# fevzibabaoglu/adaptive-edge-aware-jpeg

Hardware: AMD Instinct MI355X
Metric: megapixels/sec encode (Canny+quadtree+DCT+quant), 4K batch (higher is better)
Workload: dtype f32; 1 GPU; 64 x 3840x2160 float32 RGB per GPU, YCbCr, blocks 4-64, quality 40-80 (BASELINE config 4: 512 4K images / 8 GPUs); images_per_gpu=64, height=2160, width=3840, color_space=YCbCr, steps_in_flight=4

## Files before the change

### adaptive_edge_aware_jpeg_amd/_lib.py

```python
import ctypes
import os
import threading

import numpy as np

_HERE = os.path.dirname(os.path.abspath(__file__))
LIB_PATH = os.environ.get("AEJ_LIBRARY") or os.path.join(_HERE, "libaejpeg_hip.so")

SPACE_IDS = {"YCbCr": 0, "YCoCg": 1, "YCoCg-R": 2, "OKLAB": 3, "ICtCp": 4, "ICaCb": 5, "JzAzBz": 6}
CONVERT_IDS = dict(SPACE_IDS, XYZ=7)

AEJ_ERR_ARG, AEJ_ERR_HIP, AEJ_ERR_STATE, AEJ_ERR_CAPACITY, AEJ_ERR_UNSUPPORTED = -1, -2, -3, -4, -5


class AejError(RuntimeError):
    pass


class AejPlan(ctypes.Structure):
    _fields_ = [
        ("batch", ctypes.c_int32), ("H", ctypes.c_int32), ("W", ctypes.c_int32),
        ("layer_h", ctypes.c_int32 * 3), ("layer_w", ctypes.c_int32 * 3), ("root_size", ctypes.c_int32 * 3),
        ("coeff_off", ctypes.c_int64 * 3), ("coeff_stride", ctypes.c_int64),
        ("leaf_off", ctypes.c_int64 * 3), ("leaf_stride", ctypes.c_int64),
        ("state_off", ctypes.c_int64 * 3), ("state_stride", ctypes.c_int64),
        ("workspace_bytes", ctypes.c_uint64),
    ]


_lib = None
_lib_lock = threading.Lock()

HIP_DEFAULT_HW_QUEUES = 4
_hw_queues = HIP_DEFAULT_HW_QUEUES
_hw_queues_source = "HIP default (assumed)"


def _look_at_hw_queues():
    global _hw_queues, _hw_queues_source
    present = os.environ.get("GPU_MAX_HW_QUEUES")
    if present is not None:
        try:
            v = int(present)
        except ValueError:
            v = 0
        if v > 0:
            _hw_queues, _hw_queues_source = v, "GPU_MAX_HW_QUEUES was in the environment when the package was imported"
    return _hw_queues


def configure_hw_queues(want=16):
    global _hw_queues, _hw_queues_source
    import sys
    if os.environ.get("GPU_MAX_HW_QUEUES") is not None:
        return _look_at_hw_queues()
    trusted = "torch" not in sys.modules
    os.environ["GPU_MAX_HW_QUEUES"] = str(int(want))
    if trusted:
        _hw_queues, _hw_queues_source = int(want), "configure_hw_queues() before torch was imported"
        for ctx in _contexts.values():
            ctx.check(ctx.lib.aej_set_hw_queues(ctx.handle, _hw_queues))
    return _hw_queues


def set_hw_queues(n):
    global _hw_queues, _hw_queues_source
    _hw_queues, _hw_queues_source = int(n), "stated by the application (set_hw_queues)"
    for ctx in _contexts.values():
        ctx.check(ctx.lib.aej_set_hw_queues(ctx.handle, _hw_queues))


def hw_queues():
    return _hw_queues, _hw_queues_source


_warned_queue_limited = False


def warn_if_queue_limited(ctx, batch, H, W):
    global _warned_queue_limited
    if _warned_queue_limited:
        return
    sch = ctx.schedule(batch, H, W)
    if sch["limited_by_hw_queues"]:
        _warned_queue_limited = True
        import warnings
        warnings.warn(f"adaptive_edge_aware_jpeg_amd: this call ({batch} x {W}x{H}) would run as more overlapping sub-batches with more hardware "
                      f"queues; the library schedules for {sch['hw_queues']} ({_hw_queues_source}).  Put GPU_MAX_HW_QUEUES=16 into the environment "
                      "(or call adaptive_edge_aware_jpeg_amd.configure_hw_queues()) before `import torch`, or state the runtime's real value with "
                      "set_hw_queues().", RuntimeWarning, stacklevel=3)


_P, _I, _I64, _U64 = ctypes.c_void_p, ctypes.c_int, ctypes.c_int64, ctypes.c_uint64
class CannyParams(ctypes.Structure):
    _fields_ = [("canny_low_ratio", ctypes.c_double), ("canny_high_ratio", ctypes.c_double), ("clahe_clip_limit", ctypes.c_double),
                ("bilateral_sigma_color", ctypes.c_double), ("bilateral_sigma_space", ctypes.c_double), ("use_l2_gradient", ctypes.c_int)]


class JpegDecHuff(ctypes.Structure):
    _fields_ = [("lut", ctypes.c_uint16 * 512), ("maxcode", ctypes.c_int32 * 18), ("valoff", ctypes.c_int32 * 18), ("vals", ctypes.c_uint8 * 256)]


class JfifManyDesc(ctypes.Structure):
    _fields_ = [("src_offset", ctypes.c_int64), ("width", ctypes.c_int32), ("height", ctypes.c_int32), ("quality", ctypes.c_int32),
                ("components", ctypes.c_int32)]


class JpegDecDesc(ctypes.Structure):
    _fields_ = [("width", ctypes.c_int32), ("height", ctypes.c_int32), ("ncomp", ctypes.c_int32), ("hs", ctypes.c_int32), ("vs", ctypes.c_int32),
                ("mcux", ctypes.c_int32), ("mcuy", ctypes.c_int32), ("blocks_per_mcu", ctypes.c_int32), ("restart_interval", ctypes.c_int32),
                ("n_segments", ctypes.c_int32), ("sof", ctypes.c_int32), ("precision16", ctypes.c_int32),
                ("comp_id", ctypes.c_uint8 * 4), ("comp_h", ctypes.c_uint8 * 4), ("comp_v", ctypes.c_uint8 * 4), ("comp_tq", ctypes.c_uint8 * 4),
                ("qt", (ctypes.c_uint16 * 64) * 3), ("dc", JpegDecHuff * 3), ("ac", JpegDecHuff * 3),
                ("scan_offset", ctypes.c_int64), ("scan_length", ctypes.c_int64)]


class JpegProgFrame(ctypes.Structure):
    _fields_ = [("width", ctypes.c_int32), ("height", ctypes.c_int32), ("ncomp", ctypes.c_int32), ("hs", ctypes.c_int32), ("vs", ctypes.c_int32),
                ("mcux", ctypes.c_int32), ("mcuy", ctypes.c_int32), ("blocks_per_mcu", ctypes.c_int32), ("sof", ctypes.c_int32),
                ("precision16", ctypes.c_int32), ("n_scans", ctypes.c_int32), ("n_levels", ctypes.c_int32),
                ("comp_id", ctypes.c_uint8 * 4), ("comp_h", ctypes.c_uint8 * 4), ("comp_v", ctypes.c_uint8 * 4), ("comp_tq", ctypes.c_uint8 * 4),
                ("qt", (ctypes.c_uint16 * 64) * 3)]


class JpegProgScan(ctypes.Structure):
    _fields_ = [("ncomp", ctypes.c_int32), ("comp", ctypes.c_int32 * 4), ("td", ctypes.c_int32 * 4), ("ta", ctypes.c_int32 * 4),
                ("ss", ctypes.c_int32), ("se", ctypes.c_int32), ("ah", ctypes.c_int32), ("al", ctypes.c_int32),
                ("restart_interval", ctypes.c_int32), ("units_x", ctypes.c_int32), ("units_y", ctypes.c_int32),
                ("n_segments", ctypes.c_int32), ("level", ctypes.c_int32), ("dc", JpegDecHuff * 3), ("ac", JpegDecHuff),
                ("data_offset", ctypes.c_int64), ("data_length", ctypes.c_int64)]


class ResampleDesc(ctypes.Structure):
    _fields_ = [("src_offset", ctypes.c_int64), ("dst_offset", ctypes.c_int64), ("src_w", ctypes.c_int32), ("src_h", ctypes.c_int32),
                ("dst_w", ctypes.c_int32), ("dst_h", ctypes.c_int32), ("box", ctypes.c_float * 4), ("filter", ctypes.c_int32),
                ("reduce_x", ctypes.c_int32), ("reduce_y", ctypes.c_int32), ("reduce_box", ctypes.c_int32 * 4), ("reserved", ctypes.c_int32)]


SIGNATURES = {
    "aej_abi_version": (_I, []),
    "aej_create": (_P, [_I, _P]),
    "aej_destroy": (None, [_P]),
    "aej_last_error": (ctypes.c_char_p, [_P]),
    "aej_synchronize": (_I, [_P]),
    "aej_set_stream": (_I, [_P, _P]),
    "aej_get_hysteresis_stats": (_I, [_P, _P]),
    "aej_set_graph_mode": (_I, [_P, _I]),
    "aej_set_sub_batches": (_I, [_P, _I]),
    "aej_set_hw_queues": (_I, [_P, _I]),
    "aej_get_schedule_host": (_I, [_P, _I, _I, _I, _P]),
    "aej_set_option": (_I, [_P, ctypes.c_char_p, _I64]),
    "aej_get_option": (_I, [_P, ctypes.c_char_p, _P]),
    "aej_test_fail_after_stage": (_I, [_P, _I]),
    "aej_encode_batch_begin": (_I, [_P, _P, _I, _I, _I, _I, _P, _P, _P, _P, _P, _P, _U64]),
    "aej_encode_batch_end": (_I, [_P]),
    "aej_get_split_calls": (ctypes.c_int64, [_P]),
    "aej_get_graph_stats": (_I, [_P, _P]),
    "aej_set_profiling": (_I, [_P, _I]),
    "aej_get_stage_ms": (_I, [_P, _P]),
    "aej_stage_name": (ctypes.c_char_p, [_I]),
    "aej_set_settings": (_I, [_P, _I, _I, _I, _P]),
    "aej_encode_plan": (_I, [_P, _I, _I, _I, ctypes.POINTER(AejPlan)]),
    "aej_encode_batch": (_I, [_P, _P, _I, _I, _I, _P, _P, _P, _P, _P, _P, _U64]),
    "aej_encode_batch_u8": (_I, [_P, _P, _I, _I, _I, _P, _P, _P, _P, _P, _P, _U64]),
    "aej_metrics_workspace_bytes": (_U64, [_I, _I, _I]),
    "aej_metrics_batch": (_I, [_P, _P, _P, _I, _I, _I, _I, _P, _P, _U64]),
    "aej_color_convert": (_I, [_P, _I, _P, _P, _I64]),
    "aej_color_planes": (_I, [_P, _P, _I, _I, _I, _P, _P, _P]),
    "aej_canny_workspace_bytes": (_U64, [_I, _I]),
    "aej_canny": (_I, [_P, _P, _I, _I, _P, _P, _P, _P, _U64]),
    "aej_set_canny_params": (_I, [_P, _P]),
    "aej_quadtree_workspace_bytes": (_U64, [_I, _I, _I, _I]),
    "aej_quadtree_capacity": (_I, [_I, _I, _I, _I, ctypes.POINTER(_I64), ctypes.POINTER(_I64), ctypes.POINTER(_I64)]),
    "aej_quadtree": (_I, [_P, _P, _I, _I, _I, _I, _P, _P, _P, _P, _U64]),
    "aej_dct_quant_zigzag": (_I, [_P, _P, _I, _I, _I, _P, _I64, _P, _P]),
    "aej_deflate_stream_bound": (_U64, [_U64]),
    "aej_deflate_workspace_bytes": (_U64, [_P, _I, _I, _I]),
    "aej_deflate_histogram": (_I, [_P, _P, _P, _I, _I, _I, _P, _P, _U64]),
    "aej_deflate_batch": (_I, [_P, _P, _P, _I, _I, _I, _P, _I, _P, _U64, _P, _P, _U64]),
    "aej_deflate_build_tables": (_I, [_P, _P, _P]),
    "aej_pack_u8_levels_host": (_I, [_P, _I64, _P, _I]),
    "aej_decode_workspace_bytes": (_U64, [_P, _I, _I, _I]),
    "aej_decode_batch": (_I, [_P, _P, _P, _P, _I, _I, _I, _P, _P, _U64]),
    "aej_decode_batch_tables": (_I, [_P, _P, _P, _P, _I, _I, _I, _P, _P, _P, _U64]),
    "aej_requantise_batch": (_I, [_P, _P, _P, _P, _I, _I, _I, _I, _P, _P, _U64]),
    "aej_color_convert_inverse": (_I, [_P, _I, _P, _P, _I64]),
    "aej_leaf_positions_host": (_I64, [_P, _I64, _I, _I, _I, _P]),
    "aej_inflate_batch": (_I, [_P, _P, _P, _I, _P, _U64, _P, _P]),
    "aej_decode_headers_workspace_bytes": (_U64, [_P, _I, _I, _I]),
    "aej_decode_headers": (_I, [_P, _P, _P, _P, _I, _I, _I, _P, _P, _P, _P, _U64]),
    "aej_lpips_weights_bytes": (_U64, []),
    "aej_lpips_param_count": (_I64, []),
    "aej_lpips_pack_weights_host": (_I, [_P, _I64, _P]),
    "aej_lpips_features_bytes": (_U64, [_I, _I, _I]),
    "aej_lpips_workspace_bytes": (_U64, [_I, _I, _I]),
    "aej_lpips_features": (_I, [_P, _P, _P, _I, _I, _I, _P, _P, _U64]),
    "aej_lpips_batch": (_I, [_P, _P, _P, _P, _P, _I, _I, _I, _P, _P, _U64]),
    "aej_jfif_workspace_bytes": (_U64, [_I, _I, _I, _I]),
    "aej_jfif_headers_host": (_I, [_I, _I, _I, _P, _I]),
    "aej_jfif_encode_batch": (_I, [_P, _P, _I, _I, _I, _I, _P, _P, _U64, _P, _P, _P, _P, _U64]),
    "aej_jfif_recon_batch": (_I, [_P, _I, _I, _I, _I, _P, _P, _U64]),
    "aej_jfif_workspace_bytes_opt": (_U64, [_I, _I, _I, _I, _I, _I]),
    "aej_jfif_headers_host_opt": (_I, [_I, _I, _I, _I, _P, _I]),
    "aej_jfif_huffman_host": (_I, [_P, _P, _P, _I]),
    "aej_jfif_encode_batch_opt": (_I, [_P, _P, _I, _I, _I, _I, _P, _I, _I, _P, _U64, _P, _P, _P, _P, _U64]),
    "aej_jfif_recon_batch_opt": (_I, [_P, _I, _I, _I, _I, _I, _I, _P, _P, _U64]),
    "aej_jfif_workspace_bytes_prog": (_U64, [_I, _I, _I, _I, _I]),
    "aej_jfif_encode_batch_prog": (_I, [_P, _P, _I, _I, _I, _I, _P, _I, _P, _U64, _P, _P, _P, _P, _U64]),
    "aej_jfif_recon_batch_prog": (_I, [_P, _I, _I, _I, _I, _I, _P, _P, _U64]),
    "aej_test_jfif_prog_scan_host": (_I, [_P, ctypes.c_int64, _I, _I, _I, _I, _P, _U64, _P, _P, _P]),
    "aej_test_jfif_prog_scan": (_I, [_P, _P, ctypes.c_int64, _I, _I, _I, _I, _P, _U64, _P, _P, _P]),
    "aej_jpegdec_parse_host": (_I, [_P, _U64, _P, _P, _I]),
    "aej_jpegdec_workspace_bytes": (_U64, [_P, _P, _I]),
    "aej_jpegdec_batch": (_I, [_P, _P, _I, _P, _U64, _P, _P, _U64, _P, _P, _P, _U64]),
    "aej_jpegdec_sync_rounds": (_I64, [_P]),
    "aej_jpegdec_workspace_bytes_scaled": (_U64, [_P, _P, _I, _P]),
    "aej_jpegdec_batch_scaled": (_I, [_P, _P, _I, _P, _P, _U64, _P, _P, _U64, _P, _P, _P, _U64]),
    "aej_jpegprog_parse_host": (_I, [_P, _U64, _P, _P, _I, _P, _I]),
    "aej_jpegprog_workspace_bytes": (_U64, [_P, _P, _P, _I]),
    "aej_jpegprog_batch": (_I, [_P, _P, _P, _I, _P, _U64, _P, _P, _U64, _P, _P, _P, _U64]),
    "aej_jpegprog_workspace_bytes_scaled": (_U64, [_P, _P, _P, _I, _P]),
    "aej_jpegprog_batch_scaled": (_I, [_P, _P, _P, _I, _P, _P, _U64, _P, _P, _U64, _P, _P, _P, _U64]),
    "aej_jfif_transcode_headers_host": (_I, [_P, _P, _P, _I, _P, _I]),
    "aej_jfif_transcode_workspace_bytes": (_U64, [_P, _P, _I, _P, _P, _I, _I]),
    "aej_jfif_transcode_batch": (_I, [_P, _P, _I, _P, _U64, _P, _P, _P, _I, _P, _U64, _P, _P, _I, _P, _U64, _P, _P, _P, _P, _P, _P, _U64]),
    "aej_jfif_many_workspace_bytes": (_U64, [_P, _P, _I, _I, _I, _I]),
    "aej_jfif_many_encode": (_I, [_P, _P, _I, _P, _U64, _I, _I, _I, _P, _U64, _P, _P, _P, _P, _P, _U64]),
    "aej_jfif_many_coefs_host": (_I64, [_I, _I, _I, _I, _P, _P, _I64]),
    "aej_jfif_headers_grey_host": (_I, [_I, _I, _I, _P, _I]),
    "aej_jfif_many_coefs_grey_host": (_I64, [_I, _I, _I, _P, _P, _I64]),
    "aej_jfif_transform_geometry_host": (_I, [_I, _I, _I, _I, _I, _I, _P]),
    "aej_jfif_transform_coefs_host": (_I64, [_I, _I, _I, _I, _I, _I, _P, _I64, _P, _I64]),
    "aej_jfif_transform_coefs_grey_host": (_I64, [_I, _I, _I, _I, _P, _I64, _P, _I64]),
    "aej_jfif_transform_headers_host": (_I, [_P, _P, _P, _I, _I, _I, _P, _I]),
    "aej_jfif_transform_workspace_bytes": (_U64, [_P, _P, _I, _P, _P, _I, _I, _P, _I]),
    "aej_jfif_transform_batch": (_I, [_P, _P, _I, _P, _U64, _P, _P, _P, _I, _P, _U64, _P, _P, _I, _P, _I, _P, _U64, _P, _P, _P, _P, _P, _P, _U64]),
    "aej_resample_taps_host": (_I, [_I, ctypes.c_float, ctypes.c_float, _I, _I, _P, _P, _I64]),
    "aej_resample_workspace_bytes": (_U64, [_P, _P, _I]),
    "aej_resample_batch": (_I, [_P, _P, _I, _P, _U64, _P, _U64, _P, _U64]),
    "aej_test_jpegprog_coefs": (_I, [_P, _P, _P, _I, _P, _U64, _P, _I, _P, _U64, _P, _P, _U64]),
    "aej_test_jpegprog_coefs_host": (_I, [_P, _P, _P, _U64, _I, _P, _U64]),
    "aej_test_jpegdec_idct_host": (_I, [_P, _P, _I, _P]),
}

INFLATE_STATUS = ["ok", "bad zlib header", "bad block type", "bad code lengths", "invalid literal/length or distance code",
                  "distance too far back", "stored block LEN/NLEN mismatch", "truncated stream", "output over capacity",
                  "Adler-32 mismatch", "bad stream descriptor"]
JPEGDEC_STATUS = ["ok", "truncated scan (it ends before the last MCU)", "bad Huffman code", "coefficient run past 63",
                  "DC category above 11", "restart marker out of sequence, missing or unexpected",
                  "coefficient out of range for an 8-bit JPEG (AC beyond +-1023 or DC outside -1024..1023)"]
HEADER_STATUS = ["ok", "more leaves than the layer holds", "leaf size outside the block-size range of the header",
                 "quadtree header does not tile the layer", "coefficient count does not match the quadtree header", "bad layer descriptor"]


def load_library():
    global _lib
    with _lib_lock:
        if _lib is None:
            if not os.path.exists(LIB_PATH):
                raise AejError(
                    f"{LIB_PATH} is missing: build it with `python -c 'import __graft_entry__ as g; g.build()'` "
                    "(hipcc --offload-arch=gfx950).  There is no CPU fallback.")
            import torch
            lib = ctypes.CDLL(LIB_PATH)
            for name, (res, args) in SIGNATURES.items():
                fn = getattr(lib, name)
                fn.restype = res
                fn.argtypes = args
            _lib = lib
    return _lib


def _torch():
    import torch
    if not torch.cuda.is_available():
        raise AejError("no HIP device visible to PyTorch-ROCm: the adaptive-JPEG encode path runs on the GPU only")
    return torch


class Context:

    def __init__(self, device=0):
        self.torch = _torch()
        self.lib = load_library()
        self.device = self.torch.device("cuda", device if isinstance(device, int) else device.index or 0)
        self.stream = self.torch.cuda.current_stream(self.device).cuda_stream
        self.handle = self.lib.aej_create(self.device.index, ctypes.c_void_p(self.stream))
        if not self.handle:
            raise AejError(self.lib.aej_last_error(None).decode())
        self.check(self.lib.aej_set_hw_queues(self.handle, _hw_queues))
        self.settings_key = None
        self._ws = None

    def check_stream(self):
        cur = self.torch.cuda.current_stream(self.device).cuda_stream
        if cur != self.stream:
            raise AejError(f"context bound to stream {self.stream:#x} used while torch's current stream is {cur:#x}: "
                           "obtain the context with get_context() inside the `torch.cuda.stream(...)` block")

    def __del__(self):
        try:
            if getattr(self, "handle", None):
                self.lib.aej_destroy(self.handle)
                self.handle = None
        except Exception:
# ... 122 lines not shown
```

### adaptive_edge_aware_jpeg_amd/csrc/aej_common.h

```cpp
#pragma once
#include <hip/hip_runtime.h>
#include <stdint.h>

namespace aej {

constexpr int kMaxSizes = 8;
constexpr int kClaheTiles = 4;
constexpr int kHystTile = 64;
constexpr int kBlurTW = 64, kBlurTH = 32;
constexpr int kQtChunk = 256;

struct Geom {
    int B;
    int nl;
    int H, W;
    int h[3], w[3];
    int rh[3], rw[3];
    long long poff[3];
    long long pstride;
    int tiled;
    int ctw[3], cth[3];
    int wpr[3];
    long long bpoff[3];
    long long bpstride;
};

struct QtGeom {
    int bmin, bmax;
    int cell;
    int root[3];
    int ncell[3];
    int ltot[3];
    long long pyr_off[3];
    long long pyr_stride;
    int nchunk[3];
    long long chunk_off[3];
    long long chunk_stride;
    long long coeff_off[3], coeff_stride;
    long long leaf_off[3], leaf_stride;
    long long state_off[3], state_stride;
    long long coeff_cap[3], leaf_cap[3], state_cap[3];
    int nsizes;
    long long work_off[3][kMaxSizes], work_stride[kMaxSizes];
};
struct Tuning {
    int color_strip = 1;
    int color_strip_rows = 0;
    int color_workgroups = 0;
    int planes_row_major = 0;
    int dct64_kernel = 0;
    int dct_small_workgroups = 0;
    int sobel_lds = 0;
    int dct_multi = 1;
    int sobel_xcd = 1;
};

#define AEJ_ZIGZAG_8X8                                                                                                                      \
    0, 1, 8, 16, 9, 2, 3, 10, 17, 24, 32, 25, 18, 11, 4, 5, 12, 19, 26, 33, 40, 48, 41, 34, 27, 20, 13, 6, 7, 14, 21, 28, 35, 42, 49, 56, 57, \
        50, 43, 36, 29, 22, 15, 23, 30, 37, 44, 51, 58, 59, 52, 45, 38, 31, 39, 46, 53, 60, 61, 54, 47, 55, 62, 63

constexpr int kChunkInts = 4 + kMaxSizes;
constexpr int kMaxPlanes = 3072;

constexpr int kMetricBand = 32;

struct LeafWork {
    unsigned xy;
    int coef;
};
__host__ __device__ __forceinline__ LeafWork pack_work(int x, int y, int coef)
{
    LeafWork w;
    w.xy = (unsigned)x | ((unsigned)y << 16);
    w.coef = coef;
    return w;
}
__device__ __forceinline__ int4 unpack_work(int plane, const LeafWork &w) { return make_int4(plane, (int)(w.xy & 0xffffu), (int)(w.xy >> 16), w.coef); }

struct DctTables {
    const float *D[kMaxSizes];
    const int *zzinv[kMaxSizes];
    const int *qm[3][kMaxSizes];
};

__host__ __device__ inline long long plane_elem(int tiled, int w, int y, int x)
{
    return tiled ? ((long long)(y >> 2) * (w >> 2) + (x >> 2)) * 16 + ((y & 3) << 2) + (x & 3) : (long long)y * w + x;
}

__host__ __device__ inline long long bp_index(int y, int xw, int wpr) { return ((long long)(y >> 6) * wpr + xw) * 64 + (y & 63); }
__host__ __device__ inline long long bp_words(int h, int wpr) { return (long long)((h + 63) / 64) * wpr * 64; }

inline int ilog2(int v) { int l = 0; while ((1 << l) < v) l++; return l; }

__device__ __forceinline__ int wave_scan_incl(int v)
{
    v += __builtin_amdgcn_update_dpp(0, v, 0x111, 0xf, 0xf, false);
    v += __builtin_amdgcn_update_dpp(0, v, 0x112, 0xf, 0xf, false);
    v += __builtin_amdgcn_update_dpp(0, v, 0x114, 0xf, 0xf, false);
    v += __builtin_amdgcn_update_dpp(0, v, 0x118, 0xf, 0xf, false);
    v += __builtin_amdgcn_update_dpp(0, v, 0x142, 0xa, 0xf, false);
    v += __builtin_amdgcn_update_dpp(0, v, 0x143, 0xc, 0xf, false);
    return v;
}
__device__ __forceinline__ unsigned wave_max_u32(unsigned v)
{
    auto mx = [](unsigned a, int b) { return a > (unsigned)b ? a : (unsigned)b; };
    v = mx(v, __builtin_amdgcn_update_dpp(0, (int)v, 0x111, 0xf, 0xf, false));
    v = mx(v, __builtin_amdgcn_update_dpp(0, (int)v, 0x112, 0xf, 0xf, false));
    v = mx(v, __builtin_amdgcn_update_dpp(0, (int)v, 0x114, 0xf, 0xf, false));
    v = mx(v, __builtin_amdgcn_update_dpp(0, (int)v, 0x118, 0xf, 0xf, false));
    v = mx(v, __builtin_amdgcn_update_dpp(0, (int)v, 0x142, 0xa, 0xf, false));
    v = mx(v, __builtin_amdgcn_update_dpp(0, (int)v, 0x143, 0xc, 0xf, false));
    return (unsigned)__builtin_amdgcn_readlane((int)v, 63);
}
__device__ __forceinline__ int wave_total(int v) { return __builtin_amdgcn_readlane(wave_scan_incl(v), 63); }

}

#define AEJ_HIP_CHECK(expr)                                                       \
    do {                                                                          \
        hipError_t _e = (expr);                                                   \
        if (_e != hipSuccess) return aej::hip_fail(ctx, _e, #expr, __FILE__, __LINE__); \
    } while (0)
```

### adaptive_edge_aware_jpeg_amd/csrc/aej_ctx.h

```cpp
#pragma once
#include <math.h>
#include <stdarg.h>
#include <stdio.h>
#include <string.h>

#include <algorithm>
#include <atomic>
#include <mutex>
#include <string>
#include <thread>
#include <vector>

#include "../../include/aej.h"
#include "../../include/aej_testing.h"
#include "aej_common.h"
#include "aej_launch.h"

struct aej_pending;
constexpr int kFlagWords = 16;
constexpr int kMaxDevices = 64;
struct aej_ctx {
    int device = 0;
    hipStream_t stream = nullptr;
    std::string err;
    bool has_settings = false;
    int space = 0, bmin = 0, bmax = 0, nsizes = 0;
    void *tables = nullptr;
    const float *d_D[aej::kMaxSizes] = {};
    const int *d_zzinv[aej::kMaxSizes] = {};
    const int *d_zz[aej::kMaxSizes] = {};
    const int *d_qm[3][aej::kMaxSizes] = {};
    int *d_check = nullptr;
    const float *d_space_w = nullptr, *d_color_w = nullptr;
    float *d_bilateral = nullptr;
    aej_canny_params canny = { 0.10, 0.30, 0.75, 75.0, 75.0, 1 };
    int *h_flag = nullptr;
    long long last_hyst_queued = 0;
    bool capturing = false;
    long long n_encode_calls = 0;
    int graph_mode = 0;
    hipStream_t gstream = nullptr;
    hipEvent_t gevent = nullptr;
    struct GraphEntry {
        const void *rgb; void *coeffs, *leaves, *states, *counts, *dct, *ws;
        int batch, H, W, in_u8;
        hipGraphExec_t exec;
        unsigned long long last_use;
    };
    std::vector<GraphEntry> graphs;
    unsigned long long graph_clock = 0, n_graph_launches = 0, n_graph_captures = 0;
    int sub_mode = 0;
    int hw_queues = 4;
    int fail_after = -1;
    static constexpr int kMaxSub = 8;
    int dct_crowded = 0;
    hipStream_t sub_stream[kMaxSub] = {};
    hipEvent_t sub_color_done[kMaxSub] = {}, sub_in = nullptr;
    int *sub_flag[kMaxSub] = {};
    long long n_split_calls = 0;
    int sub_chain = -1;
    int chain_hook = 0;
    hipEvent_t chain_event = nullptr;
    aej::Tuning tune;
    int jd_subseq_bits = 2048;
    long long jd_sync_rounds = 0;
    struct aej_pending *pending = nullptr;
    bool profiling = false;
    hipEvent_t ev[24] = {};
    int ev_stage[24] = {};
    int n_ev = 0;
    float stage_ms[AEJ_N_STAGES] = {};
};

namespace aej {
inline int fail(aej_ctx *ctx, int code, const char *fmt, ...)
{
    char buf[512];
    va_list ap;
    va_start(ap, fmt);
    vsnprintf(buf, sizeof buf, fmt, ap);
    va_end(ap);
    if (ctx) ctx->err = buf;
    return code;
}
int hip_fail(aej_ctx *ctx, hipError_t e, const char *expr, const char *file, int line);

inline bool is_pow2(int v) { return v > 0 && (v & (v - 1)) == 0; }
inline long long align_up(long long v, long long a) { return (v + a - 1) / a * a; }

struct Carver {
    char *base;
    unsigned long long off = 0;
    explicit Carver(void *p) : base(static_cast<char *>(p)) {}
    template <typename T> T *take(long long n)
    {
        off = (off + 255) & ~255ull;
        T *p = base ? reinterpret_cast<T *>(base + off) : nullptr;
        off += (unsigned long long)n * sizeof(T);
        return p;
    }
    unsigned long long bytes() const { return (off + 255) & ~255ull; }
};

}

extern const double kMid[7][3], kScale[7][3];
int check_encode_args(aej_ctx *ctx, int batch, int H, int W);
int make_geom(aej_ctx *ctx, int space, int B, int H, int W, aej::Geom &g);
void make_plane_geom(int H, int W, aej::Geom &g);
int make_qtgeom(aej_ctx *ctx, const aej::Geom &g, int bmin, int bmax, aej::QtGeom &q, bool allow_small_root = false);
int make_geoms(aej_ctx *ctx, int batch, int H, int W, aej::Geom &g, aej::QtGeom &q);
long long big_scratch_floats(int bmax);

bool call_in_flight(const aej_ctx *ctx);
void drop_graphs(aej_ctx *ctx);
void release_encode_state(aej_ctx *ctx);

#define AEJ_TRY(expr) do { const int _rc = (expr); if (_rc) return _rc; } while (0)

inline int refuse_in_flight(aej_ctx *ctx, const char *fn)
{
    return call_in_flight(ctx) ? aej::fail(ctx, AEJ_ERR_STATE, "%s between aej_encode_batch_begin and aej_encode_batch_end", fn) : 0;
}
inline int enter(aej_ctx *ctx, const char *fn) { return ctx ? refuse_in_flight(ctx, fn) : AEJ_ERR_ARG; }
inline int bind_device(aej_ctx *ctx) { AEJ_HIP_CHECK(hipSetDevice(ctx->device)); return 0; }
inline int check_workspace(aej_ctx *ctx, unsigned long long need, uint64_t got)
{
    return need > got ? aej::fail(ctx, AEJ_ERR_CAPACITY, "workspace too small: need %llu bytes, got %llu", need, (unsigned long long)got) : 0;
}
inline int null_buffer(aej_ctx *ctx, const char *fn = nullptr)
{
    return fn ? aej::fail(ctx, AEJ_ERR_ARG, "%s: NULL buffer", fn) : aej::fail(ctx, AEJ_ERR_ARG, "NULL buffer");
}
inline void copy_msg(const std::string &m, char *msg, int msg_capacity)
{
    if (!msg || msg_capacity < 1) return;
    const size_t k = std::min(m.size(), (size_t)msg_capacity - 1);
    memcpy(msg, m.data(), k);
    msg[k] = 0;
}
```

### adaptive_edge_aware_jpeg_amd/csrc/aej_launch.h

```cpp
#pragma once
#include "aej_common.h"

namespace aej {

int launch_color_convert(hipStream_t st, int space, const float *rgb, float *out, long long n);
bool color_planes_can_tile(const Geom &g, int space, bool in_u8, const Tuning &t);
int launch_color_planes(hipStream_t st, int space, const void *rgb, bool in_u8, const Geom &g, const float *mid, const float *scale,
                        float *raw, float *norm, unsigned char *u8, int *tile_hist, const Tuning &t);
struct AreaTabs {
    int mode;
    int isx, isy;
    const int *xoff, *xsi, *yoff, *ysi;
    const float *xal, *yal;
};
int launch_color_planes_generic(hipStream_t st, int space, const void *rgb, bool in_u8, const Geom &g, const float *mid, const float *scale,
                                const AreaTabs &tabs, float *raw, float *norm, unsigned char *u8, int *tile_hist);
void launch_plane_u8(hipStream_t st, const float *plane, const Geom &g, unsigned char *u8, int *tile_hist);

struct CannyBuffers {
    unsigned char *u8a;
    unsigned char *u8b;
    int *tile_hist;
    unsigned char *lut;
    int *blur_hist;
    int *thr;
    unsigned long long *weak;
    unsigned long long *strong;
    int *hflags;
    int *hlist;
    int *pass_count;
    const float *space_w;
    const float *color_w;
    double low_q = 0.10 * 100, high_q = 0.30 * 100;
    double clip_limit = 0.75;
    int l2 = 1;
    unsigned char *dump_clahe, *dump_gauss;
};
constexpr int kHystCounters = 128;
long long hyst_tiles_per_image(const Geom &g);
int hyst_ring_slots(const Geom &g);
void launch_clahe_pad_hist(hipStream_t st, const Geom &g, const CannyBuffers &cb);
void launch_clahe_lut(hipStream_t st, const Geom &g, const CannyBuffers &cb);
void launch_clahe_blur(hipStream_t st, const Geom &g, const CannyBuffers &cb);
void launch_thresholds(hipStream_t st, const Geom &g, const CannyBuffers &cb);
void launch_sobel_nms(hipStream_t st, const Geom &g, const CannyBuffers &cb, const Tuning &t);
void launch_hysteresis(hipStream_t st, const Geom &g, const CannyBuffers &cb);
void launch_zero(hipStream_t st, void *p16, size_t bytes_multiple_of_16);
void launch_bits_to_edge(hipStream_t st, const Geom &g, const unsigned long long *strong, unsigned char *edge01);
void launch_bits_to_map(hipStream_t st, const Geom &g, const unsigned long long *weak, const unsigned long long *strong, unsigned char *map);

struct QtBuffers {
    unsigned char *pyr;
    const unsigned long long *edge_bits;
    int *chunk_cnt;
    unsigned short *lane_code;
    int *leaves;
    unsigned char *states;
    long long *counts;
    LeafWork *work[kMaxSizes];
    int *work_count;
    long long work_cap[kMaxSizes];
    int *overflow;
};
void launch_qt_cells(hipStream_t st, const Geom &g, const QtGeom &q, const unsigned long long *edge_bits, const QtBuffers &qb);
void launch_pack_edge_bits(hipStream_t st, const Geom &g, const unsigned char *edge, unsigned long long *bits);
void launch_qt_count(hipStream_t st, const Geom &g, const QtGeom &q, const QtBuffers &qb);
void launch_qt_scan(hipStream_t st, const Geom &g, const QtGeom &q, const QtBuffers &qb);
void launch_qt_emit(hipStream_t st, const Geom &g, const QtGeom &q, const QtBuffers &qb);

constexpr int kBigBlocks = 128;
constexpr int kMaxBlock = 1024;
constexpr int big_blocks(int S) { return S <= 256 ? kBigBlocks : S == 512 ? 64 : 32; }
constexpr long long big_scratch_floats_for(int S) { return S >= 256 ? (long long)big_blocks(S) * S * S : 0; }
struct DctArgs {
    const float *norm;
    int *coeffs;
    float *dct_f32;
    const LeafWork *work;
    float *scratch;
    const int *work_count;
    int k;
    int nplanes;
    const float *D;
    const int *zzinv;
    const int *qm[3];
    int crowded = 0;
};
int launch_dct(hipStream_t st, int size, const Geom &g, const QtGeom &q, const DctArgs &a, long long max_items, const Tuning &t);
int launch_dct_multi(hipStream_t st, const Geom &g, const QtGeom &q, const DctArgs *args, const long long *max_items);
void launch_work_from_leaves(hipStream_t st, const int *leaves, long long n, int bmin, int plane, LeafWork *const *work, int *work_count);


struct IdctArgs {
    const int *coeffs;
    float *planes;
    const LeafWork *work;
    float *scratch;
    const int *work_count;
    int k, nplanes;
    const float *D;
    const int *zz, *zzinv;
    const int *qm[3];
    float mid[3], scale[3];
};
void launch_work_from_tables(hipStream_t st, const Geom &g, const QtGeom &q, const int *leaves, const long long *counts, LeafWork *const *work,
                             int *work_count, int *bad );
int launch_idct(hipStream_t st, int size, const Geom &g, const QtGeom &q, const IdctArgs &a, long long max_items);
int launch_color_inverse(hipStream_t st, int space, const float *in, float *out, long long n);
int launch_upsample_color(hipStream_t st, int space, const Geom &g, const float *planes, float *rgb);

unsigned long long deflate_stream_bound(unsigned long long raw_bytes);
unsigned long long deflate_workspace_bytes(int batch, const long long *coeff_cap );
void launch_deflate_parse(hipStream_t st, const int *coeffs, const long long *counts, int batch, long long coeff_stride, const long long *coeff_off,
                          const long long *coeff_cap, int *hist, void *workspace);
void launch_deflate(hipStream_t st, const int *coeffs, const long long *counts, int batch, long long coeff_stride, const long long *coeff_off,
                    const long long *coeff_cap, const unsigned *tables , int reuse_parse, unsigned char *out,
                    unsigned long long stream_stride, long long *sizes, void *workspace);

void launch_inflate(hipStream_t st, const unsigned char *src, const long long *desc, int n, unsigned char *dst, long long dst_bytes,
                    long long *out_bytes, int *status);

struct HdrGeom {
    int bmin, bmax;
    int h[3], w[3];
    int proot[3];
    long long leaf_off[3], leaf_span[3], leaf_stride;
    long long coeff_span[3];
};
void launch_headers(hipStream_t st, const unsigned char *states, const long long *desc, const long long *inflated, int nlayers, const HdrGeom &g,
                    unsigned char *codes, int *leaves, long long *counts, int *status);

void launch_requant_check(hipStream_t st, const Geom &g, const QtGeom &q, const int *leaves, const long long *counts, const int *qmats,
                          long long qmat_words, int *bad);
int launch_requant(hipStream_t st, const Geom &g, const QtGeom &q, const float *dct, const int *leaves, const long long *counts, int n_sets,
                   const int *qmats, const int *const *zz, int *out, long long set_stride, int *bad, int blocks_per_plane);

struct MetricParts {
    long long stride;
    int psnr_n;
    long long grey_off, grey_n;
    long long lvl_off[5], lvl_n[5];
};
int metric_prep_blocks(long long npx);
long long ssim_partials(int h, int w);
void launch_metric_prep(hipStream_t st, const float *a, const float *b, int B, long long npx, double *part, long long stride, unsigned char *ga,
                        unsigned char *gb);
void launch_metric_pool_grey(hipStream_t st, const unsigned char *ga, const unsigned char *gb, int B, int H, int W, int f, int hp, int wp, float *xa,
                             float *xb);
void launch_ssim_level(hipStream_t st, bool interleaved, const float *xa, const float *xb, int B, int C, int h, int w, const float *g11, double *part,
                       long long stride, long long off, bool want_ss, float *pool_a = nullptr, float *pool_b = nullptr);
void launch_pool2_rgb(hipStream_t st, const float *ia, const float *ib, int B, int h, int w, int p, int h2, int w2, float *oa, float *ob);
void launch_pool2(hipStream_t st, bool interleaved, const float *in, int B, int C, int h, int w, int p, int h2, int w2, float *out);
void launch_metric_final(hipStream_t st, const double *part, const MetricParts &P, int B, long long npx, long long n_ssim, const long long *n_level, double *out);


constexpr int kLpipsTaps = 5;
constexpr int kLpipsHeadPixels = 256;
struct LpipsLayer { int cin, cinp, cout, k, stride, pad; };
extern const LpipsLayer kLpipsLayers[kLpipsTaps];
struct LpipsGeom {
    int H, W;
    int h[kLpipsTaps], w[kLpipsTaps];
    int ph[2], pw[2];
    long long tap_off[kLpipsTaps];
    long long feat_elems;
    long long x_elems, y_elems;
    int nblk[kLpipsTaps], max_blk;
};
bool lpips_geom(int H, int W, LpipsGeom &g);
long long lpips_param_floats();
long long lpips_packed_floats(long long off[kLpipsTaps][3]);
void lpips_pack_host(const float *params, float *packed);
void launch_lpips(hipStream_t st, const float *wpk, const float *img, int B, const LpipsGeom &g, float *X, float *Y, float *feats_out,
                  const float *feats_a, double *partial, double *out);


constexpr int kJfifBlockWords = 52;
constexpr int kJfifBlockWordsOpt = 53;
constexpr int kJfifHdrMax = 1024;
struct JfifGeom {
    int B, H, W, nq;
    int mcux, mcuy, ybx, yby;
    int yw, yh, cw, ch;
    long long n_mcu, nblk;
    long long stream_words, n_chunks;
    long long plane_bytes;
    int hs, vs, opt, ncomp;
};
struct JfifParams {
    int qt[2][64];
    int hdr_len, dht_off, pad_[2];
    unsigned char hdr[kJfifHdrMax];
};
struct JfifBufs {
    JfifParams *par; int *dct; short *coef; int *lens; long long *boff, *btot; unsigned *stream; int *ffcnt; long long *ffpre, *fftot, *total;
    unsigned char *planes;
    unsigned long long *hist; unsigned *codes; unsigned char *fhdr; int *fhdr_len;
};
bool jfif_geom(int B, int H, int W, int nq, JfifGeom &g, int ss = 2, int opt = 0, int ncomp = 3);
unsigned long long jfif_carve(void *base, const JfifGeom &g, JfifBufs &w);
void jfif_quant_tables(int q, int luma[64], int chroma[64]);
void jfif_params_host(int q, int H, int W, JfifParams &p, int ss = 2, int ncomp = 3);
constexpr int jfif_sof_bytes(int ncomp) { return 10 + 3 * ncomp; }
constexpr int jfif_sos_bytes(int ncomp) { return 8 + 2 * ncomp; }
int jfif_huffman_host(const long long *counts, unsigned char *bits, unsigned char *huffval);
hipError_t launch_jfif_encode(hipStream_t st, const JfifGeom &g, const JfifBufs &w, const JfifParams *par_host, const unsigned char *rgb,
                              unsigned char *out, unsigned long long cap, long long *lengths, long long *offsets);
hipError_t launch_jfif_recon(hipStream_t st, const JfifGeom &g, const JfifBufs &w, unsigned char *rgb_out);
hipError_t launch_jfif_coefs(hipStream_t st, const JfifGeom &g, const JfifBufs &w, const JfifParams *par_host, const unsigned char *rgb);

struct Carver;
unsigned long long jfif_carve_coded(Carver &c, const JfifGeom &g, JfifBufs &w);
hipError_t launch_jfif_entropy(hipStream_t st, const JfifGeom &g, const JfifBufs &w, long long *lengths, long long *offsets);
hipError_t launch_jfif_entropy_annexk(hipStream_t st, const JfifGeom &g, const JfifBufs &w, long long *lengths, long long *offsets);
hipError_t launch_jfif_scatter(hipStream_t st, const JfifGeom &g, const JfifBufs &w, const long long *lengths, const long long *offsets,
                               unsigned char *out, unsigned long long cap);

constexpr int kJfpMaxScans = 10;
constexpr int kJfpPiece = 576;
struct JfpScan {
    int Ss, Se, Ah, Al;
    int comp, tbl;
    long long n, ioff;
    long long woff, wcap, coff;
};
struct JfpGeom {
    int segs, hs, vs, nchroma;
    int mcux, ybx, nscan, ntab;
    int raw, B;
    long long nblk, T, nmax;
    long long stream_words, n_chunks;
    JfpScan sc[kJfpMaxScans];
};
struct JfpBufs {
    unsigned short *flags;
    unsigned long long *pre;
    int *plen, *lens;
    unsigned *stream; int *ffcnt; unsigned long long *ffpre;
// ... 209 lines not shown
```

### adaptive_edge_aware_jpeg_amd/csrc/api.hip

```cpp
#include "aej_ctx.h"

using namespace aej;

int aej::hip_fail(aej_ctx *ctx, hipError_t e, const char *expr, const char *file, int line)
{
    return fail(ctx, AEJ_ERR_HIP, "%s failed: %s (%s:%d)", expr, hipGetErrorString(e), file, line);
}

static const int kRatios[7][3][2] = {
    { { 1, 1 }, { 2, 2 }, { 2, 2 } },
    { { 1, 1 }, { 2, 2 }, { 2, 2 } },
    { { 1, 1 }, { 2, 2 }, { 2, 2 } },
    { { 1, 1 }, { 2, 2 }, { 2, 2 } },
    { { 1, 1 }, { 1, 4 }, { 1, 4 } },
    { { 1, 1 }, { 1, 4 }, { 1, 4 } },
    { { 1, 1 }, { 2, 2 }, { 2, 2 } },
};
const double kMid[7][3] = {
    { 0.5000000037252903, 7.450580596923828e-09, 0.0 }, { 0.5, 0.0, 0.0 }, { 0.5, 0.0, 0.0 },
    { 0.4999999, 0.021152213, -0.056563325 }, { 0.07497266, -0.0008235276, 0.023989676 },
    { 0.07498085, 0.02180194, -0.018250957 }, { 0.0087900255, 0.00048353244, -0.0020741792 },
};
const double kScale[7][3] = {
    { 253.99999810755253, 254.000003784895, 254.0 }, { 254.0, 254.0, 254.0 }, { 254.0, 127.0, 127.0 },
// ... 45 lines not shown
        off += align_up((long long)g.h[l] * g.w[l], 64);
    }
    g.pstride = off;
    fill_clahe_geom(g);
    return 0;
}

void make_plane_geom(int H, int W, Geom &g)
{
    memset(&g, 0, sizeof g);
    g.B = 1; g.nl = 1; g.H = H; g.W = W;
    g.h[0] = H; g.w[0] = W; g.rh[0] = g.rw[0] = 1;
    g.poff[0] = 0;
    g.pstride = align_up((long long)H * W, 64);
    fill_clahe_geom(g);
}

int make_qtgeom(aej_ctx *ctx, const Geom &g, int bmin, int bmax, QtGeom &q, bool allow_small_root)
{
    memset(&q, 0, sizeof q);
    if (!is_pow2(bmin) || !is_pow2(bmax) || bmin > bmax || bmin < 1)
        return fail(ctx, AEJ_ERR_ARG, "block sizes must be powers of two with min <= max (got %d, %d)", bmin, bmax);
    q.bmin = bmin; q.bmax = bmax; q.cell = bmin;
    long long pyr = 0, chunks = 0, co = 0, lo = 0, so = 0;
    for (int l = 0; l < g.nl; l++) {
        int root = root_size_of(g.h[l], g.w[l]);
        if (root < bmin) {
            if (!allow_small_root || g.nl != 1) return fail(ctx, AEJ_ERR_UNSUPPORTED, "layer %d (%dx%d): root %d smaller than min block %d", l, g.h[l], g.w[l], root, bmin);
            q.cell = root;
        }
        q.root[l] = root;
        q.ncell[l] = root / q.cell;
        q.ltot[l] = ilog2(q.ncell[l]);
        if (q.ltot[l] > 14) return fail(ctx, AEJ_ERR_UNSUPPORTED, "quadtree deeper than 14 levels");
        q.pyr_off[l] = pyr;
        long long states = 0;
        for (int j = 0; j <= q.ltot[l]; j++) { long long s = q.ncell[l] >> j; states += s * s; }
        pyr += align_up(states, 256);
        long long nc2 = (long long)q.ncell[l] * q.ncell[l];
        q.nchunk[l] = (int)(nc2 / 256 > 0 ? nc2 / 256 : 1);
        q.chunk_off[l] = chunks;
        chunks += q.nchunk[l];
        int top = bmax < root ? bmax : root;
        long long wc = align_up(g.w[l], top), hc = align_up(g.h[l], top);
        if (wc > root) wc = root;
        if (hc > root) hc = root;
        q.coeff_cap[l] = wc * hc;
        q.leaf_cap[l] = (wc / q.cell) * (hc / q.cell);
        q.state_cap[l] = states;
        q.coeff_off[l] = co; co += align_up(q.coeff_cap[l], 64);
        q.leaf_off[l] = lo;  lo += align_up(q.leaf_cap[l], 16);
        q.state_off[l] = so; so += align_up(q.state_cap[l], 64);
    }
    q.pyr_stride = pyr; q.chunk_stride = chunks;
    q.coeff_stride = co; q.leaf_stride = lo; q.state_stride = so;
    int k = 0;
    for (int s = bmin; s <= bmax && k < kMaxSizes; s *= 2, k++) {
        long long off = 0;
        for (int l = 0; l < g.nl; l++) {
            q.work_off[l][k] = off;
            if (s > q.root[l]) continue;
            int top = bmax < q.root[l] ? bmax : q.root[l];
            long long wc = align_up(g.w[l], top), hc = align_up(g.h[l], top);
            if (wc > q.root[l]) wc = q.root[l];
            if (hc > q.root[l]) hc = q.root[l];
            off += ((wc + s - 1) / s) * ((hc + s - 1) / s);
        }
        q.work_stride[k] = off;
    }
    q.nsizes = k;
    return 0;
}

long long big_scratch_floats(int bmax)
{
    long long m = 0;
    for (int s = 256; s <= bmax; s *= 2) m = std::max(m, big_scratch_floats_for(s));
    return m;
}

int check_encode_args(aej_ctx *ctx, int batch, int H, int W)
{
    if (!ctx) return AEJ_ERR_ARG;
    if (!ctx->has_settings) return fail(ctx, AEJ_ERR_STATE, "aej_set_settings has not been called");
    if (batch < 1 || H < 1 || W < 1) return fail(ctx, AEJ_ERR_ARG, "batch, H, W must be positive");
    if (batch * 3 > kMaxPlanes) return fail(ctx, AEJ_ERR_UNSUPPORTED, "batch %d too large for one call (max %d images)", batch, kMaxPlanes / 3);
    return 0;
}

int make_geoms(aej_ctx *ctx, int batch, int H, int W, Geom &g, QtGeom &q)
{
    AEJ_TRY(make_geom(ctx, ctx->space, batch, H, W, g));
    return make_qtgeom(ctx, g, ctx->bmin, ctx->bmax, q);
}

extern "C" int aej_abi_version(void) { return AEJ_ABI_VERSION; }

extern "C" aej_ctx *aej_create(int device, void *hip_stream)
{
    int n = 0;
    if (hipGetDeviceCount(&n) != hipSuccess || device < 0 || device >= n || device >= kMaxDevices) return nullptr;
    if (hipSetDevice(device) != hipSuccess) return nullptr;
    aej_ctx *ctx = new aej_ctx();
    ctx->device = device;
    ctx->stream = static_cast<hipStream_t>(hip_stream);
    if (hipHostMalloc(reinterpret_cast<void **>(&ctx->h_flag), kFlagWords * sizeof(int), hipHostMallocDefault) != hipSuccess) { delete ctx; return nullptr; }
    return ctx;
}

extern "C" void aej_destroy(aej_ctx *ctx)
{
    if (!ctx) return;
    (void)bind_device(ctx);
    release_encode_state(ctx);
    if (ctx->gstream) (void)hipStreamDestroy(ctx->gstream);
    if (ctx->gevent) (void)hipEventDestroy(ctx->gevent);
    if (ctx->tables) (void)hipFree(ctx->tables);
    if (ctx->d_bilateral) (void)hipFree(ctx->d_bilateral);
    for (int i = 0; i < aej_ctx::kMaxSub; i++) {
        if (ctx->sub_stream[i]) (void)hipStreamDestroy(ctx->sub_stream[i]);
        if (ctx->sub_color_done[i]) (void)hipEventDestroy(ctx->sub_color_done[i]);
        if (ctx->sub_flag[i]) (void)hipHostFree(ctx->sub_flag[i]);
    }
    if (ctx->sub_in) (void)hipEventDestroy(ctx->sub_in);
    if (ctx->h_flag) (void)hipHostFree(ctx->h_flag);
    for (int i = 0; i < 24; i++) if (ctx->ev[i]) (void)hipEventDestroy(ctx->ev[i]);
    delete ctx;
}

extern "C" const char *aej_last_error(aej_ctx *ctx)
{
    if (!ctx) return "aej: no context (aej_create failed: no such HIP device?)";
    return ctx->err.c_str();
}

extern "C" int aej_synchronize(aej_ctx *ctx)
{
    AEJ_TRY(enter(ctx, __func__));
    AEJ_HIP_CHECK(hipStreamSynchronize(ctx->stream));
    return 0;
}

static void zigzag_order(int s, std::vector<int> &zz)
{
    zz.resize((size_t)s * s);
    int i = 0;
    for (int d = 0; d < 2 * s - 1; d++) {
        int lo = d - s + 1 > 0 ? d - s + 1 : 0, hi = d < s - 1 ? d : s - 1;
        if (d % 2) for (int r = lo; r <= hi; r++) zz[i++] = r * s + (d - r);
        else for (int r = hi; r >= lo; r--) zz[i++] = r * s + (d - r);
    }
}

extern "C" int aej_set_settings(aej_ctx *ctx, int space, int bmin, int bmax, const int32_t *qmats_host)
{
    AEJ_TRY(enter(ctx, __func__));
    if (space < 0 || space > 6) return fail(ctx, AEJ_ERR_ARG, "Unsupported color space id: %d", space);
    if (!is_pow2(bmin) || !is_pow2(bmax) || bmin > bmax || bmin < 2)
        return fail(ctx, AEJ_ERR_ARG, "block size range (%d, %d): powers of two with 2 <= min <= max required", bmin, bmax);
    if (bmax > kMaxBlock)
        return fail(ctx, AEJ_ERR_UNSUPPORTED, "block size range (%d, %d): no kernel for blocks above %d", bmin, bmax, kMaxBlock);
    if (ilog2(bmax) - ilog2(bmin) + 1 > kMaxSizes)
        return fail(ctx, AEJ_ERR_UNSUPPORTED, "block size range (%d, %d) spans more than %d sizes", bmin, bmax, kMaxSizes);
    if (!qmats_host) return fail(ctx, AEJ_ERR_ARG, "qmats_host is NULL");
    AEJ_TRY(bind_device(ctx));
    int nsizes = 0;
    for (int s = bmin; s <= bmax; s *= 2) nsizes++;
    std::vector<char> blob;
    auto put = [&](const void *p, size_t bytes) {
        size_t o = (blob.size() + 255) & ~(size_t)255;
        blob.resize(o + bytes);
        memcpy(blob.data() + o, p, bytes);
        return o;
    };
    size_t oD[kMaxSizes], oZ[kMaxSizes], oZf[kMaxSizes], oQ[3][kMaxSizes];
    int k = 0;
    size_t qpos = 0;
    std::vector<size_t> qoff_layer_size;
    for (int s = bmin; s <= bmax; s *= 2, k++) {
        std::vector<float> D((size_t)s * s);
        for (int u = 0; u < s; u++) {
            double alpha = u == 0 ? sqrt(1.0 / (double)s) : sqrt(2.0 / (double)s);
            for (int n = 0; n < s; n++) D[(size_t)u * s + n] = (float)(alpha * cos(3.14159265358979323846 * (double)(2 * n + 1) * (double)u / (2.0 * (double)s)));
        }
        oD[k] = put(D.data(), D.size() * 4);
        std::vector<int> zz, inv((size_t)s * s);
        zigzag_order(s, zz);
        for (int i = 0; i < s * s; i++) inv[zz[i]] = i;
        oZ[k] = put(inv.data(), inv.size() * 4);
        oZf[k] = put(zz.data(), zz.size() * 4);
    }
    for (int l = 0; l < 3; l++) {
        k = 0;
        for (int s = bmin; s <= bmax; s *= 2, k++) {
            for (int i = 0; i < s * s; i++)
                if (qmats_host[qpos + i] < 1) return fail(ctx, AEJ_ERR_ARG, "quantisation matrix entries must be >= 1");
            oQ[l][k] = put(qmats_host + qpos, (size_t)s * s * 4);
            qpos += (size_t)s * s;
        }
    }
    const int zero_words[64] = {};
    const size_t oCheck = put(zero_words, sizeof zero_words);
    drop_graphs(ctx);
    if (ctx->tables) { AEJ_HIP_CHECK(hipStreamSynchronize(ctx->stream)); AEJ_HIP_CHECK(hipFree(ctx->tables)); ctx->tables = nullptr; }
    AEJ_HIP_CHECK(hipMalloc(&ctx->tables, blob.size()));
    AEJ_HIP_CHECK(hipMemcpy(ctx->tables, blob.data(), blob.size(), hipMemcpyHostToDevice));
    char *base = static_cast<char *>(ctx->tables);
    for (int i = 0; i < kMaxSizes; i++) {
        ctx->d_D[i] = nullptr; ctx->d_zzinv[i] = nullptr; ctx->d_zz[i] = nullptr;
        for (int l = 0; l < 3; l++) ctx->d_qm[l][i] = nullptr;
    }
    for (int i = 0; i < nsizes; i++) {
        ctx->d_D[i] = reinterpret_cast<const float *>(base + oD[i]);
        ctx->d_zzinv[i] = reinterpret_cast<const int *>(base + oZ[i]);
        ctx->d_zz[i] = reinterpret_cast<const int *>(base + oZf[i]);
        for (int l = 0; l < 3; l++) ctx->d_qm[l][i] = reinterpret_cast<const int *>(base + oQ[l][i]);
    }
    ctx->d_check = reinterpret_cast<int *>(base + oCheck);
    ctx->space = space; ctx->bmin = bmin; ctx->bmax = bmax; ctx->nsizes = nsizes;
    ctx->has_settings = true;
    return 0;
}

extern "C" int aej_set_canny_params(aej_ctx *ctx, const aej_canny_params *p)
{
    AEJ_TRY(enter(ctx, __func__));
    const aej_canny_params def = { 0.10, 0.30, 0.75, 75.0, 75.0, 1 };
    const aej_canny_params v = p ? *p : def;
    if (!(v.canny_low_ratio >= 0.0 && v.canny_low_ratio <= 1.0 && v.canny_high_ratio >= 0.0 && v.canny_high_ratio <= 1.0))
        return fail(ctx, AEJ_ERR_ARG, "Canny threshold ratios must lie in [0, 1] (np.percentile takes 0..100)");
    if (!(v.clahe_clip_limit == v.clahe_clip_limit) || !(v.bilateral_sigma_color == v.bilateral_sigma_color) || !(v.bilateral_sigma_space == v.bilateral_sigma_space))
        return fail(ctx, AEJ_ERR_ARG, "NaN Canny hyper-parameter");
    const bool tables_change = v.bilateral_sigma_color != ctx->canny.bilateral_sigma_color || v.bilateral_sigma_space != ctx->canny.bilateral_sigma_space;
    ctx->canny = v;
    drop_graphs(ctx);
    if (tables_change) { ctx->d_color_w = nullptr; ctx->d_space_w = nullptr; }
    return 0;
}

extern "C" int aej_get_hysteresis_stats(aej_ctx *ctx, int64_t *out_host)
{
    if (!ctx || !out_host) return AEJ_ERR_ARG;
    out_host[0] = ctx->n_encode_calls;
    out_host[1] = ctx->last_hyst_queued;
    return 0;
}

extern "C" int aej_set_graph_mode(aej_ctx *ctx, int mode)
{
    if (!ctx || mode < 0 || mode > 2) return AEJ_ERR_ARG;
    AEJ_TRY(refuse_in_flight(ctx, __func__));
    ctx->graph_mode = mode;
    if (mode == 0) drop_graphs(ctx);
    return 0;
}

extern "C" int aej_set_sub_batches(aej_ctx *ctx, int n)
{
    if (!ctx || n < 0 || n > aej_ctx::kMaxSub) return AEJ_ERR_ARG;
    ctx->sub_mode = n;
    return 0;
}

extern "C" int64_t aej_get_split_calls(aej_ctx *ctx) { return ctx ? (int64_t)ctx->n_split_calls : -1; }

extern "C" int aej_set_hw_queues(aej_ctx *ctx, int n)
{
    if (!ctx || n < 1) return AEJ_ERR_ARG;
    ctx->hw_queues = n;
    return 0;
}

namespace {
struct OptionDef { const char *name; int aej::Tuning::*field; int aej_ctx::*ctx_field; long long lo, hi; bool drops_graphs; };
const OptionDef kOptions[] = {
    { "color_strip", &aej::Tuning::color_strip, nullptr, 0, 1, true },
    { "color_strip_rows", &aej::Tuning::color_strip_rows, nullptr, 0, 64, true },
    { "color_workgroups", &aej::Tuning::color_workgroups, nullptr, 0, 1 << 16, true },
    { "planes_row_major", &aej::Tuning::planes_row_major, nullptr, 0, 1, true },
    { "dct64_kernel", &aej::Tuning::dct64_kernel, nullptr, 0, 4, true },
    { "dct_small_workgroups", &aej::Tuning::dct_small_workgroups, nullptr, 0, 1 << 16, true },
    { "sobel_lds", &aej::Tuning::sobel_lds, nullptr, 0, 1, true },
    { "sobel_xcd", &aej::Tuning::sobel_xcd, nullptr, 0, 1, true },
    { "dct_multi", &aej::Tuning::dct_multi, nullptr, 0, 1, true },
    { "sub_chain", nullptr, &aej_ctx::sub_chain, -1, 3, false },
    { "jpegdec_subseq_bits", nullptr, &aej_ctx::jd_subseq_bits, 32, 1 << 20, false },
};
const OptionDef *find_option(const char *name)
{
    if (!name) return nullptr;
    for (const OptionDef &o : kOptions) if (!strcmp(o.name, name)) return &o;
    return nullptr;
}
}

extern "C" int aej_set_option(aej_ctx *ctx, const char *name, int64_t value)
{
    AEJ_TRY(enter(ctx, __func__));
    const OptionDef *o = find_option(name);
    if (!o) return fail(ctx, AEJ_ERR_ARG, "aej_set_option: unknown option '%s'", name ? name : "(null)");
    if (value < o->lo || value > o->hi || (o->field == &aej::Tuning::dct64_kernel && value != 0 && value != 1 && value != 4))
        return fail(ctx, AEJ_ERR_ARG, "aej_set_option: %s = %lld outside its range [%lld, %lld]", name, (long long)value, o->lo, o->hi);
    if (o->field) ctx->tune.*(o->field) = (int)value;
    else ctx->*(o->ctx_field) = (int)value;
    if (o->drops_graphs) drop_graphs(ctx);
    return 0;
}

extern "C" int aej_get_option(aej_ctx *ctx, const char *name, int64_t *value_host)
{
    if (!ctx || !value_host) return AEJ_ERR_ARG;
    const OptionDef *o = find_option(name);
    if (!o) return fail(ctx, AEJ_ERR_ARG, "aej_get_option: unknown option '%s'", name ? name : "(null)");
    *value_host = o->field ? ctx->tune.*(o->field) : ctx->*(o->ctx_field);
    return 0;
}

extern "C" int aej_test_fail_after_stage(aej_ctx *ctx, int stage)
{
    if (!ctx || stage < -1 || stage >= AEJ_N_STAGES) return AEJ_ERR_ARG;
    ctx->fail_after = stage;
    return 0;
}

extern "C" int aej_get_graph_stats(aej_ctx *ctx, int64_t *out_host)
{
    if (!ctx || !out_host) return AEJ_ERR_ARG;
    out_host[0] = (int64_t)ctx->n_graph_launches;
    out_host[1] = (int64_t)ctx->n_graph_captures;
    out_host[2] = (int64_t)ctx->graphs.size();
    return 0;
}

extern "C" int aej_set_stream(aej_ctx *ctx, void *hip_stream)
{
    AEJ_TRY(enter(ctx, __func__));
    hipStream_t s = static_cast<hipStream_t>(hip_stream);
    if (s == ctx->stream) return 0;
    AEJ_TRY(bind_device(ctx));
    AEJ_HIP_CHECK(hipStreamSynchronize(ctx->stream));
    ctx->stream = s;
    return 0;
}

extern "C" int aej_set_profiling(aej_ctx *ctx, int enable)
{
    AEJ_TRY(enter(ctx, __func__));
    ctx->profiling = enable != 0;
    return 0;
}

extern "C" int aej_get_stage_ms(aej_ctx *ctx, float *ms_host)
{
    if (!ctx || !ms_host) return AEJ_ERR_ARG;
    for (int i = 0; i < AEJ_N_STAGES; i++) ms_host[i] = ctx->stage_ms[i];
    return 0;
}

extern "C" const char *aej_stage_name(int i)
{
    static const char *names[AEJ_N_STAGES] = { "clear", "color_planes", "clahe_lut", "clahe_blur", "thresholds", "sobel_nms",
                                               "hysteresis", "quadtree", "dct2", "dct4", "dct8", "dct16", "dct32", "dct64", "dct128", "dct256", "dct512", "dct1024" };
    return i >= 0 && i < AEJ_N_STAGES ? names[i] : "";
}
```

### adaptive_edge_aware_jpeg_amd/csrc/api_encode.hip

```cpp
#include "aej_ctx.h"

using namespace aej;

static void mark(aej_ctx *ctx, int stage)
{
    if (!ctx->profiling || ctx->n_ev >= 24) return;
    if (!ctx->ev[ctx->n_ev] && hipEventCreate(&ctx->ev[ctx->n_ev]) != hipSuccess) return;
    ctx->ev_stage[ctx->n_ev] = stage;
    (void)hipEventRecord(ctx->ev[ctx->n_ev], ctx->stream);
    ctx->n_ev++;
}

static int injected_failure(aej_ctx *ctx, int stage)
{
    if (ctx->fail_after != stage) return 0;
    ctx->fail_after = -1;
    ctx->err = std::string("injected failure after stage ") + aej_stage_name(stage);
    return AEJ_ERR_STATE;
}

static void collect_marks(aej_ctx *ctx)
{
    for (int i = 0; i < AEJ_N_STAGES; i++) ctx->stage_ms[i] = 0.f;
    for (int i = 1; i < ctx->n_ev; i++) {
// ... 134 lines not shown
{
    hipStream_t st = ctx->stream;
    if (ctx->capturing) launch_zero(st, w.zero_begin, (size_t)(w.zero_end - w.zero_begin));
    else AEJ_HIP_CHECK(hipMemsetAsync(w.zero_begin, 0, (size_t)(w.zero_end - w.zero_begin), st));
    w.qb.edge_bits = edge_bits;
    launch_qt_cells(st, g, q, edge_bits, w.qb);
    launch_qt_count(st, g, q, w.qb);
    launch_qt_scan(st, g, q, w.qb);
    launch_qt_emit(st, g, q, w.qb);
    AEJ_HIP_CHECK(hipGetLastError());
    return 0;
}

static void area_tab(int ssize, int dsize, double scale, std::vector<int> &off, std::vector<int> &si, std::vector<float> &alpha)
{
    off.assign((size_t)dsize + 1, 0); si.clear(); alpha.clear();
    for (int dx = 0; dx < dsize; dx++) {
        double fsx1 = dx * scale, fsx2 = fsx1 + scale;
        double cell = scale < ssize - fsx1 ? scale : ssize - fsx1;
        int sx1 = (int)ceil(fsx1), sx2 = (int)floor(fsx2);
        if (sx2 > ssize - 1) sx2 = ssize - 1;
        if (sx1 > sx2) sx1 = sx2;
        off[dx] = (int)si.size();
        if (sx1 - fsx1 > 1e-3) { si.push_back(sx1 - 1); alpha.push_back((float)((sx1 - fsx1) / cell)); }
        for (int sx = sx1; sx < sx2; sx++) { si.push_back(sx); alpha.push_back((float)(1.0 / cell)); }
        if (fsx2 - sx2 > 1e-3) {
            double a = fsx2 - sx2;
            if (a > 1.) a = 1.;
            if (a > cell) a = cell;
            si.push_back(sx2); alpha.push_back((float)(a / cell));
        }
    }
    off[dsize] = (int)si.size();
}

static long long area_tab_ints(const Geom &g)
{
    return 2LL * (g.w[1] + 1 + g.h[1] + 1) + 2LL * (g.W + 2 * g.w[1] + 2) + 2LL * (g.H + 2 * g.h[1] + 2) + 64;
}

static bool planes_fast_ok(const Geom &g)
{
    bool ok = (g.W % 4) == 0 && (g.H % 2) == 0;
    for (int l = 1; l < 3; l++) ok = ok && g.h[l] * g.rh[l] == g.H && g.w[l] * g.rw[l] == g.W;
    return ok;
}

static int run_color_planes(aej_ctx *ctx, const void *rgb, bool in_u8, const Geom &g, float *raw, float *norm, unsigned char *u8, int *hist,
                            int *tab_ws)
{
    float mid[3], scale[3];
    for (int i = 0; i < 3; i++) { mid[i] = (float)kMid[ctx->space][i]; scale[i] = (float)kScale[ctx->space][i]; }
    if (planes_fast_ok(g)) {
        Tuning t = ctx->tune;
        if (t.color_workgroups == 0 && ctx->dct_crowded && ctx->space < 3) t.color_workgroups = 224;
        if (launch_color_planes(ctx->stream, ctx->space, rgb, in_u8, g, mid, scale, raw, norm, u8, hist, t)) return fail(ctx, AEJ_ERR_ARG, "bad colour space");
        return 0;
    }
    AreaTabs t;
    memset(&t, 0, sizeof t);
    double sx = 1.0 / ((double)g.w[1] / (double)g.W), sy = 1.0 / ((double)g.h[1] / (double)g.H);
    int isx = (int)lrint(sx), isy = (int)lrint(sy);
    bool fast = fabs(sx - isx) < 2.220446049250313e-16 && fabs(sy - isy) < 2.220446049250313e-16;
    t.isx = isx; t.isy = isy;
    if (fast) t.mode = (isx == 2 && isy == 2) ? 0 : 1;
    else {
        t.mode = 2;
        if (!tab_ws) return fail(ctx, AEJ_ERR_STATE, "no workspace for the INTER_AREA tables");
        std::vector<int> xoff, xsi, yoff, ysi;
        std::vector<float> xal, yal;
        area_tab(g.W, g.w[1], sx, xoff, xsi, xal);
        area_tab(g.H, g.h[1], sy, yoff, ysi, yal);
        std::vector<int> blob;
        auto put_i = [&](const std::vector<int> &v) { size_t o = blob.size(); blob.insert(blob.end(), v.begin(), v.end()); return o; };
        auto put_f = [&](const std::vector<float> &v) { size_t o = blob.size(); blob.resize(o + v.size()); memcpy(blob.data() + o, v.data(), v.size() * 4); return o; };
        size_t o1 = put_i(xoff), o2 = put_i(xsi), o3 = put_f(xal), o4 = put_i(yoff), o5 = put_i(ysi), o6 = put_f(yal);
        if ((long long)blob.size() > area_tab_ints(g)) return fail(ctx, AEJ_ERR_CAPACITY, "INTER_AREA tables larger than reserved");
        AEJ_HIP_CHECK(hipMemcpyAsync(tab_ws, blob.data(), blob.size() * 4, hipMemcpyHostToDevice, ctx->stream));
        AEJ_HIP_CHECK(hipStreamSynchronize(ctx->stream));
        t.xoff = tab_ws + o1; t.xsi = tab_ws + o2; t.xal = reinterpret_cast<const float *>(tab_ws + o3);
        t.yoff = tab_ws + o4; t.ysi = tab_ws + o5; t.yal = reinterpret_cast<const float *>(tab_ws + o6);
    }
    if (launch_color_planes_generic(ctx->stream, ctx->space, rgb, in_u8, g, mid, scale, t, raw, norm, u8, hist)) return fail(ctx, AEJ_ERR_ARG, "bad colour space");
    return 0;
}

struct EncodeWs {
    float *big;
    float *norm;
    int *area_tabs;
    CannyWs canny;
    QtWs qt;
    unsigned long long bytes;
};

static void carve_encode(void *base, const Geom &g, const QtGeom &q, EncodeWs &w)
{
    Carver c(base);
    w.norm = c.take<float>((long long)g.B * g.pstride);
    w.area_tabs = c.take<int>(area_tab_ints(g));
    carve_canny(c, g, w.canny);
    carve_qt(c, g, q, true, w.qt);
    w.big = big_scratch_floats(q.bmax) ? c.take<float>(big_scratch_floats(q.bmax)) : nullptr;
    w.bytes = c.bytes();
}

static unsigned long long sub_ws_bytes(Geom g, const QtGeom &q, int nsub)
{
    g.B = (g.B + nsub - 1) / nsub;
    EncodeWs w;
    carve_encode(nullptr, g, q, w);
    return w.bytes;
}

extern "C" int aej_encode_plan(aej_ctx *ctx, int batch, int H, int W, aej_plan *plan)
{
    AEJ_TRY(check_encode_args(ctx, batch, H, W));
    if (!plan) return fail(ctx, AEJ_ERR_ARG, "plan is NULL");
    Geom g;
    QtGeom q;
    AEJ_TRY(make_geoms(ctx, batch, H, W, g, q));
    EncodeWs w;
    carve_encode(nullptr, g, q, w);
    memset(plan, 0, sizeof *plan);
    plan->batch = batch; plan->H = H; plan->W = W;
    for (int l = 0; l < 3; l++) {
        plan->layer_h[l] = g.h[l]; plan->layer_w[l] = g.w[l]; plan->root_size[l] = q.root[l];
        plan->coeff_off[l] = q.coeff_off[l]; plan->leaf_off[l] = q.leaf_off[l]; plan->state_off[l] = q.state_off[l];
    }
    plan->coeff_stride = q.coeff_stride; plan->leaf_stride = q.leaf_stride; plan->state_stride = q.state_stride;
    plan->workspace_bytes = w.bytes;
    for (int n = 2; n <= aej_ctx::kMaxSub && n <= batch; n++)
        plan->workspace_bytes = std::max<uint64_t>(plan->workspace_bytes, sub_ws_bytes(g, q, n) * (unsigned long long)n);
    return 0;
}

constexpr long long kGraphAutoPixels = 8LL << 20;

static int enqueue_back(aej_ctx *ctx, const Geom &g, const QtGeom &q, EncodeWs &w, int32_t *coeffs, float *dct_f32)
{
    hipStream_t st = ctx->stream;
    AEJ_TRY(run_quadtree(ctx, g, q, w.qt, w.canny.cb.strong));
    mark(ctx, AEJ_STAGE_QUADTREE);
    DctArgs args[kMaxSizes];
    int k = 0;
    for (int s = q.bmin; s <= q.bmax; s *= 2, k++) {
        DctArgs &a = args[k];
        a.norm = w.norm; a.coeffs = coeffs; a.dct_f32 = dct_f32;
        a.work = w.qt.qb.work[k]; a.work_count = w.qt.qb.work_count; a.k = k; a.nplanes = g.B * 3;
        a.scratch = w.big;
        a.D = ctx->d_D[k]; a.zzinv = ctx->d_zzinv[k];
        a.crowded = ctx->dct_crowded;
        for (int l = 0; l < 3; l++) a.qm[l] = ctx->d_qm[l][k];
    }
    const bool one_launch = ctx->tune.dct_multi && !ctx->profiling && (long long)g.B * g.H * g.W <= kGraphAutoPixels;
    if (!(one_launch && launch_dct_multi(st, g, q, args, w.qt.qb.work_cap) == 0)) {
        k = 0;
        for (int s = q.bmin; s <= q.bmax; s *= 2, k++) {
            if (launch_dct(st, s, g, q, args[k], w.qt.qb.work_cap[k], ctx->tune)) return fail(ctx, AEJ_ERR_UNSUPPORTED, "no DCT kernel for block size %d with %d planes", s, args[k].nplanes);
            mark(ctx, AEJ_STAGE_DCT_2 + ilog2(s) - 1);
        }
    }
    AEJ_HIP_CHECK(hipGetLastError());
    return 0;
}

static int enqueue_readback(aej_ctx *ctx, EncodeWs &w)
{
    AEJ_HIP_CHECK(hipMemcpyAsync(ctx->h_flag, w.qt.qb.overflow, sizeof(int), hipMemcpyDeviceToHost, ctx->stream));
    AEJ_HIP_CHECK(hipMemcpyAsync(ctx->h_flag + 1, w.canny.cb.pass_count + 32 , sizeof(int), hipMemcpyDeviceToHost, ctx->stream));
    return 0;
}

constexpr size_t kMaxGraphs = 8;

static int encode_graph(aej_ctx *ctx, const void *rgb, bool in_u8, const Geom &g, const QtGeom &q, EncodeWs &w, int32_t *coeffs, int32_t *leaves,
                        uint8_t *states, int64_t *counts, float *dct_f32, void *workspace, bool &used)
{
    used = false;
    if (!ctx->gstream) {
        AEJ_HIP_CHECK(hipStreamCreateWithFlags(&ctx->gstream, hipStreamNonBlocking));
        AEJ_HIP_CHECK(hipEventCreateWithFlags(&ctx->gevent, hipEventDisableTiming));
    }
    aej_ctx::GraphEntry *hit = nullptr;
    for (auto &e : ctx->graphs)
        if (e.rgb == rgb && e.coeffs == coeffs && e.leaves == leaves && e.states == states && e.counts == counts && e.dct == dct_f32 && e.ws == workspace &&
            e.batch == g.B && e.H == g.H && e.W == g.W && e.in_u8 == (int)in_u8) { hit = &e; break; }
    hipStream_t user = ctx->stream;
    if (!hit) {
        if (ctx->graphs.size() >= kMaxGraphs) {
            size_t lru = 0;
            for (size_t i = 1; i < ctx->graphs.size(); i++) if (ctx->graphs[i].last_use < ctx->graphs[lru].last_use) lru = i;
            if (ctx->graphs[lru].exec) (void)hipGraphExecDestroy(ctx->graphs[lru].exec);
            ctx->graphs.erase(ctx->graphs.begin() + (long)lru);
        }
        ctx->graphs.push_back({ rgb, coeffs, leaves, states, counts, dct_f32, workspace, g.B, g.H, g.W, (int)in_u8, nullptr, ++ctx->graph_clock });
        return 0;
    }
    if (!hit->exec) {
        hipGraph_t graph = nullptr;
        ctx->stream = ctx->gstream;
        ctx->capturing = true;
        hipError_t e = hipStreamBeginCapture(ctx->gstream, hipStreamCaptureModeThreadLocal);
        int rc = e == hipSuccess ? 0 : hip_fail(ctx, e, "hipStreamBeginCapture", __FILE__, __LINE__);
        if (!rc) rc = clear_canny_ws(ctx, w.canny);
        if (!rc) rc = run_color_planes(ctx, rgb, in_u8, g, nullptr, w.norm, w.canny.cb.u8a, w.canny.cb.tile_hist, w.area_tabs);
        if (!rc) {
            hipStream_t st = ctx->stream;
            launch_clahe_pad_hist(st, g, w.canny.cb);
            launch_clahe_lut(st, g, w.canny.cb);
            launch_clahe_blur(st, g, w.canny.cb);
            launch_thresholds(st, g, w.canny.cb);
            launch_sobel_nms(st, g, w.canny.cb, ctx->tune);
            launch_hysteresis(st, g, w.canny.cb);
            rc = enqueue_back(ctx, g, q, w, coeffs, dct_f32);
        }
        hipError_t e2 = e == hipSuccess ? hipStreamEndCapture(ctx->gstream, &graph) : hipSuccess;
        ctx->stream = user;
        ctx->capturing = false;
        if (rc || e2 != hipSuccess || !graph) {
            if (graph) (void)hipGraphDestroy(graph);
            (void)hipGetLastError();
            return rc ? rc : 0;
        }
        hipGraphExec_t exec = nullptr;
        e = hipGraphInstantiate(&exec, graph, nullptr, nullptr, 0);
        (void)hipGraphDestroy(graph);
        if (e != hipSuccess || !exec) { (void)hipGetLastError(); return 0; }
        hit->exec = exec;
        ctx->n_graph_captures++;
    }
    hit->last_use = ++ctx->graph_clock;
    AEJ_HIP_CHECK(hipEventRecord(ctx->gevent, user));
    AEJ_HIP_CHECK(hipStreamWaitEvent(ctx->gstream, ctx->gevent, 0));
    AEJ_HIP_CHECK(hipGraphLaunch(hit->exec, ctx->gstream));
    ctx->stream = ctx->gstream;
    const int rb = enqueue_readback(ctx, w);
    ctx->stream = user;
    if (rb) return rb;
    AEJ_HIP_CHECK(hipStreamSynchronize(ctx->gstream));
    ctx->n_graph_launches++;
    used = true;
    return 0;
}

static int sub_batches(const aej_ctx *ctx, const Geom &g, int hw_queues, bool as_if_unprofiled = false)
{
    if (ctx->sub_mode == 1 || (ctx->profiling && !as_if_unprofiled) || ctx->graph_mode == 2 || !planes_fast_ok(g)) return 1;
    int n = ctx->sub_mode;
    if (n == 0) {
        const long long px = (long long)g.B * g.H * g.W;
        if (hw_queues >= 8) {
            n = (px >= (384LL << 20) && g.B >= 16) ? 4 : (px >= (64LL << 20) && g.B >= 8) ? 2 : 1;
        } else {
            bool alone;
            { std::lock_guard<std::mutex> lock(g_chain_mutex); alone = g_calls_in_flight[ctx->device] == 0; }
            n = (alone && px >= (64LL << 20) && g.B >= 8) ? 2 : 1;
        }
    }
    if (n > aej_ctx::kMaxSub) n = aej_ctx::kMaxSub;
    if (n > g.B) n = g.B;
    return n;
}

struct EncodePart { Geom g; EncodeWs w; bool whole_call = false; int32_t *coeffs = nullptr; float *dct = nullptr; hipStream_t stream = nullptr; int *flag = nullptr; bool used = false; };
struct aej_pending {
    bool active = false, complete = false;
    QtGeom q;
    std::vector<EncodePart> parts;
};

bool call_in_flight(const aej_ctx *ctx) { return ctx->pending && ctx->pending->active; }

void release_encode_state(aej_ctx *ctx)
{
    if (call_in_flight(ctx)) {
        (void)hipDeviceSynchronize();
        std::lock_guard<std::mutex> lock(g_chain_mutex);
        if (g_calls_in_flight[ctx->device] > 0) g_calls_in_flight[ctx->device]--;
    }
    delete ctx->pending;
    ctx->pending = nullptr;
    {
        std::lock_guard<std::mutex> lock(g_chain_mutex);
        for (int i = 0; i < aej_ctx::kMaxSub; i++)
            if (ctx->sub_color_done[i] && g_last_color_done[ctx->device] == ctx->sub_color_done[i]) g_last_color_done[ctx->device] = nullptr;
    }
    drop_graphs(ctx);
}

static aej_pending &pending_of(aej_ctx *ctx)
{
    if (!ctx->pending) ctx->pending = new aej_pending;
    return *ctx->pending;
}

static int enqueue_part(aej_ctx *ctx, EncodePart &p, const QtGeom &q, const void *rgb, bool in_u8, hipEvent_t done)
{
    int rc;
    mark(ctx, -1);
    AEJ_TRY(clear_canny_ws(ctx, p.w.canny));
    mark(ctx, AEJ_STAGE_CLEAR);
    const bool chain = ctx->sub_chain && done && !ctx->profiling;
    const int chain_mode = ctx->sub_chain > 0 ? ctx->sub_chain : 1;
    if (chain) {
        std::lock_guard<std::mutex> lock(g_chain_mutex);
// ... 203 lines not shown
    AEJ_TRY(bind_device(ctx));
    Geom g;
    AEJ_TRY(make_geom(ctx, ctx->space, batch, H, W, g));
    int *tabs = nullptr;
    if (!planes_fast_ok(g)) AEJ_HIP_CHECK(hipMalloc(reinterpret_cast<void **>(&tabs), (size_t)area_tab_ints(g) * 4));
    const int rc = run_color_planes(ctx, rgb, false, g, planes_raw, planes_norm, planes_u8, nullptr, tabs);
    if (tabs) { (void)hipStreamSynchronize(ctx->stream); (void)hipFree(tabs); }
    if (rc) return rc;
    AEJ_HIP_CHECK(hipGetLastError());
    return 0;
}

extern "C" uint64_t aej_canny_workspace_bytes(int H, int W)
{
    if (H < 1 || W < 1) return 0;
    Geom g;
    make_plane_geom(H, W, g);
    Carver c(nullptr);
    CannyWs w;
    carve_canny(c, g, w);
    return c.bytes();
}

extern "C" int aej_canny(aej_ctx *ctx, const float *plane, int H, int W, uint8_t *edge, uint8_t *stages, int32_t *thresholds,
                         void *workspace, uint64_t workspace_bytes)
{
    AEJ_TRY(enter(ctx, __func__));
    if (H < 1 || W < 1) return fail(ctx, AEJ_ERR_ARG, "Input array must be a 2D.");
    if (!plane || !edge || !workspace) return null_buffer(ctx);
    if (workspace_bytes < aej_canny_workspace_bytes(H, W)) return fail(ctx, AEJ_ERR_CAPACITY, "workspace too small");
    AEJ_TRY(bind_device(ctx));
    AEJ_TRY(ensure_canny_tables(ctx));
    Geom g;
    make_plane_geom(H, W, g);
    Carver c(workspace);
    CannyWs w;
    carve_canny(c, g, w);
    apply_canny_params(ctx, w.cb);
    long long n = (long long)H * W;
    if (stages) { w.cb.dump_clahe = stages + n; w.cb.dump_gauss = stages + 2 * n; }
    AEJ_TRY(clear_canny_ws(ctx, w));
    launch_plane_u8(ctx->stream, plane, g, w.cb.u8a, w.cb.tile_hist);
    hipStream_t st = ctx->stream;
    if (stages) AEJ_HIP_CHECK(hipMemcpyAsync(stages, w.cb.u8a, n, hipMemcpyDeviceToDevice, st));
    launch_clahe_pad_hist(st, g, w.cb);
    launch_clahe_lut(st, g, w.cb);
    launch_clahe_blur(st, g, w.cb);
    if (stages) AEJ_HIP_CHECK(hipMemcpyAsync(stages + 3 * n, w.cb.u8b, n, hipMemcpyDeviceToDevice, st));
    launch_thresholds(st, g, w.cb);
    if (thresholds) AEJ_HIP_CHECK(hipMemcpyAsync(thresholds, w.cb.thr, 2 * sizeof(int), hipMemcpyDeviceToDevice, st));
    launch_sobel_nms(st, g, w.cb, ctx->tune);
    Geom ge = g;
    ge.pstride = n;
    if (stages) launch_bits_to_map(st, ge, w.cb.weak, w.cb.strong, stages + 4 * n);
    launch_hysteresis(st, g, w.cb);
    launch_bits_to_edge(st, ge, w.cb.strong, edge);
    AEJ_HIP_CHECK(hipGetLastError());
    AEJ_HIP_CHECK(hipStreamSynchronize(st));
    return 0;
}

extern "C" int aej_quadtree_capacity(int H, int W, int min_size, int max_size, int64_t *leaf_cap, int64_t *state_cap, int64_t *coeff_cap)
{
    if (H < 1 || W < 1) return AEJ_ERR_ARG;
    Geom g;
    make_plane_geom(H, W, g);
    QtGeom q;
    AEJ_TRY(make_qtgeom(nullptr, g, min_size, max_size, q, true));
    if (leaf_cap) *leaf_cap = q.leaf_cap[0];
    if (state_cap) *state_cap = q.state_cap[0];
    if (coeff_cap) *coeff_cap = q.coeff_cap[0];
    return 0;
}

extern "C" uint64_t aej_quadtree_workspace_bytes(int H, int W, int min_size, int max_size)
{
    if (H < 1 || W < 1) return 0;
    Geom g;
    make_plane_geom(H, W, g);
    QtGeom q;
    if (make_qtgeom(nullptr, g, min_size, max_size, q, true)) return 0;
    Carver c(nullptr);
    QtWs w;
    carve_qt(c, g, q, false, w);
    c.take<unsigned long long>(g.bpstride);
    return c.bytes();
}

extern "C" int aej_quadtree(aej_ctx *ctx, const uint8_t *edge, int H, int W, int min_size, int max_size, int32_t *leaves,
                            uint8_t *states, int64_t *counts, void *workspace, uint64_t workspace_bytes)
{
    AEJ_TRY(enter(ctx, __func__));
    if (H < 1 || W < 1) return fail(ctx, AEJ_ERR_ARG, "Input array must be a 2D with a single channel.");
    if (!edge || !leaves || !states || !counts || !workspace) return null_buffer(ctx);
    AEJ_TRY(bind_device(ctx));
    Geom g;
    make_plane_geom(H, W, g);
    g.pstride = (long long)H * W;
    QtGeom q;
    AEJ_TRY(make_qtgeom(ctx, g, min_size, max_size, q, true));
    Carver c(workspace);
    QtWs w;
    carve_qt(c, g, q, false, w);
    unsigned long long *bits = c.take<unsigned long long>(g.bpstride);
    if (c.bytes() > workspace_bytes) return fail(ctx, AEJ_ERR_CAPACITY, "workspace too small");
    w.qb.leaves = leaves; w.qb.states = states; w.qb.counts = reinterpret_cast<long long *>(counts);
    launch_pack_edge_bits(ctx->stream, g, edge, bits);
    AEJ_TRY(run_quadtree(ctx, g, q, w, bits));
    AEJ_HIP_CHECK(hipMemcpyAsync(ctx->h_flag, w.qb.overflow, sizeof(int), hipMemcpyDeviceToHost, ctx->stream));
    AEJ_HIP_CHECK(hipStreamSynchronize(ctx->stream));
    if (*ctx->h_flag) return fail(ctx, AEJ_ERR_CAPACITY, "leaf/state capacity exceeded");
    return 0;
}

extern "C" int aej_dct_quant_zigzag(aej_ctx *ctx, const float *norm, int H, int W, int layer, const int32_t *leaves, int64_t n_leaves,
                                    int32_t *coeffs, float *dct_f32)
{
    AEJ_TRY(enter(ctx, __func__));
    if (!ctx->has_settings) return fail(ctx, AEJ_ERR_STATE, "aej_set_settings has not been called");
    if (H < 1 || W < 1 || layer < 0 || layer > 2 || n_leaves < 0) return fail(ctx, AEJ_ERR_ARG, "bad argument");
    if (H > 65535 || W > 65535) return fail(ctx, AEJ_ERR_UNSUPPORTED, "plane %dx%d: sides above 65535 pixels are not built", H, W);
    if (n_leaves == 0) return 0;
    if (!norm || !leaves || !coeffs) return null_buffer(ctx);
    AEJ_TRY(bind_device(ctx));
    hipStream_t st = ctx->stream;
    Geom g;
    memset(&g, 0, sizeof g);
    g.B = 1; g.nl = 3; g.H = H; g.W = W;
    for (int l = 0; l < 3; l++) { g.h[l] = H; g.w[l] = W; g.rh[l] = g.rw[l] = 1; g.poff[l] = 0; }
    g.pstride = (long long)H * W;
    QtGeom q;
    memset(&q, 0, sizeof q);
    q.bmin = ctx->bmin; q.bmax = ctx->bmax; q.cell = ctx->bmin; q.nsizes = ctx->nsizes;
    char *scratch = nullptr;
    size_t list_bytes = (size_t)n_leaves * sizeof(LeafWork);
    size_t total = 256 + (size_t)ctx->nsizes * ((list_bytes + 255) & ~(size_t)255);
    const size_t big_off = total;
    total += (size_t)big_scratch_floats(ctx->bmax) * sizeof(float);
    AEJ_HIP_CHECK(hipMalloc(reinterpret_cast<void **>(&scratch), total));
    int *work_count = reinterpret_cast<int *>(scratch);
    LeafWork *work[kMaxSizes] = {};
    for (int k = 0; k < ctx->nsizes; k++) work[k] = reinterpret_cast<LeafWork *>(scratch + 256 + (size_t)k * ((list_bytes + 255) & ~(size_t)255));
    hipError_t e = hipMemsetAsync(scratch, 0, 256, st);
    if (e == hipSuccess) {
        launch_work_from_leaves(st, leaves, n_leaves, ctx->bmin, layer, work, work_count);
        int k = 0;
        for (int s = ctx->bmin; s <= ctx->bmax; s *= 2, k++) {
            DctArgs a;
            a.norm = norm; a.coeffs = coeffs; a.dct_f32 = dct_f32;
            a.work = work[k]; a.work_count = work_count; a.k = k; a.nplanes = 3;
            a.scratch = big_scratch_floats(ctx->bmax) ? reinterpret_cast<float *>(scratch + big_off) : nullptr;
            a.D = ctx->d_D[k]; a.zzinv = ctx->d_zzinv[k];
            for (int l = 0; l < 3; l++) a.qm[l] = ctx->d_qm[l][k];
            if (launch_dct(st, s, g, q, a, n_leaves, ctx->tune)) { e = hipErrorInvalidValue; break; }
        }
        if (e == hipSuccess) e = hipGetLastError();
        if (e == hipSuccess) e = hipStreamSynchronize(st);
    }
    (void)hipFree(scratch);
    if (e != hipSuccess) return fail(ctx, AEJ_ERR_HIP, "aej_dct_quant_zigzag: %s", hipGetErrorString(e));
    return 0;
}

extern "C" int aej_get_schedule_host(aej_ctx *ctx, int batch, int H, int W, int32_t *out_host)
{
    AEJ_TRY(check_encode_args(ctx, batch, H, W));
    if (!out_host) return fail(ctx, AEJ_ERR_ARG, "out_host is NULL");
    Geom g;
    AEJ_TRY(make_geom(ctx, ctx->space, batch, H, W, g));
    const int n = sub_batches(ctx, g, ctx->hw_queues), n_wide = sub_batches(ctx, g, 16);
    out_host[0] = ctx->hw_queues;
    out_host[1] = n;
    out_host[2] = (ctx->hw_queues < 8 && n_wide > n) ? 1 : 0;
    out_host[3] = 0;
    return 0;
}
```

### adaptive_edge_aware_jpeg_amd/csrc/dct.hip

```cpp
#include "aej_common.h"
#include "aej_launch.h"
#include "aej_bigblock.h"
#include "aej_mfma.h"
#include "aej_quant.h"
#include <stdlib.h>

namespace aej {


__device__ __forceinline__ int reflect_pad_idx(int i, int n)
{
    if (i < n) return i;
    if (n <= 1) return 0;
    int p = 2 * (n - 1);
    int j = i % p;
    return j >= n ? p - j : j;
}

template <int S>
__device__ __forceinline__ int zigzag_pos(int r, int c)
{
    const int d = r + c;
    if (d < S) {
        const int before = d * (d + 1) / 2;
// ... 505 lines not shown
                for (int s = 0; s < 4; s++) x[s] = (row0 + (long long)s * (w >> 2) * 16)[lane_tiled];
            } else {
                const float *row0 = src + ((long long)dz * w + dy);
                const unsigned lane_rm = (unsigned)(gq * w + i);
#pragma unroll
                for (int s = 0; s < 4; s++) x[s] = (row0 + (long long)s * 4 * w)[lane_rm];
            }
        } else {
            const int hc = min(S, h - dz), wc = min(S, w - dy);
            const int col = dy + reflect_pad_idx(i, wc);
#pragma unroll
            for (int s = 0; s < 4; s++) x[s] = src[plane_elem(TILED ? 1 : 0, w, dz + reflect_pad_idx(4 * s + gq, hc), col)];
        }
    };
    Desc d0 = landed(fetch(item)), d1, d2;
    float x0[4], x1[4], x2[4];
    load_x(d0, x0);
    d1 = landed(fetch(item + 4));
    Desc dv = fetch(item + 8);
    load_x(d1, x1);
    auto step = [&](const float (&x_cur)[4], const Desc &d_cur, float (&x_fill)[4], Desc &d_fill) {
        d_fill = landed(dv);
        dv = fetch(item + 12);
        load_x(d_fill, x_fill);
        const int b = d_cur.plane / 3, layer = d_cur.plane - b * 3;
        floatx4 pacc = { 0.f, 0.f, 0.f, 0.f };
#pragma unroll
        for (int s = 0; s < 4; s++) pacc = __builtin_amdgcn_mfma_f32_16x16x4f32(x_cur[s], dB[s], pacc, 0, 0, 0);
        const auto p02 = __builtin_amdgcn_permlane32_swap(__float_as_uint(pacc[0]), __float_as_uint(pacc[2]), false, false);
        const auto p13 = __builtin_amdgcn_permlane32_swap(__float_as_uint(pacc[1]), __float_as_uint(pacc[3]), false, false);
        const unsigned p02a = p02[0], p02b = p02[1], p13a = p13[0], p13b = p13[1];
        const auto q01 = __builtin_amdgcn_permlane16_swap(p02a, p13a, false, false);
        const auto q23 = __builtin_amdgcn_permlane16_swap(p02b, p13b, false, false);
        const unsigned t0 = q01[0], t1 = q01[1], t2 = q23[0], t3 = q23[1];
        const float t[4] = { __uint_as_float(t0), __uint_as_float(t1), __uint_as_float(t2), __uint_as_float(t3) };
        floatx4 y = { 0.f, 0.f, 0.f, 0.f };
#pragma unroll
        for (int s = 0; s < 4; s++) y = __builtin_amdgcn_mfma_f32_16x16x4f32(t[s], dB[s], y, 0, 0, 0);
        const long long out_base = (long long)b * q.coeff_stride + sel(layer, lcoff[0], lcoff[1], lcoff[2]) + d_cur.coef;
        if (WANT_DCT) {
#pragma unroll
            for (int r = 0; r < 4; r++) a.dct_f32[out_base + (4 * gq + r) * S + i] = y[r];
        }
        const floatx4 qf = *reinterpret_cast<const floatx4 *>(&sQf[layer * SS + lane * 4]), rq = *reinterpret_cast<const floatx4 *>(&sQr[layer * SS + lane * 4]);
        const float ymax = __builtin_fmaxf(__builtin_fmaxf(__builtin_fabsf(y[0]), __builtin_fabsf(y[1])), __builtin_fmaxf(__builtin_fabsf(y[2]), __builtin_fabsf(y[3])));
        if (!slow_q && !__any(!(ymax < 131072.0f))) {
            float kf[4], rem[4];
            unsigned long long fix = 0;
#pragma unroll
            for (int r = 0; r < 4; r++) {
                kf[r] = __builtin_rintf(y[r] * rq[r]);
                rem[r] = __builtin_fmaf(-kf[r], qf[r], y[r]);
                const float ar = __builtin_fabsf(rem[r]);
                fix |= __builtin_amdgcn_ballot_w64(ar + ar >= qf[r]);
            }
            int ki[4];
#pragma unroll
            for (int r = 0; r < 4; r++) ki[r] = (int)kf[r];
            if (fix != 0) {
#pragma unroll
                for (int r = 0; r < 4; r++) {
                    const float ar = __builtin_fabsf(rem[r]), h = 0.5f * qf[r];
                    if (ar > h || (ar == h && (ki[r] & 1))) ki[r] += rem[r] > 0.f ? 1 : -1;
                }
            }
#pragma unroll
            for (int r = 0; r < 4; r++) out_slab[zz[r]] = ki[r];
        } else {
#pragma unroll
            for (int r = 0; r < 4; r++) out_slab[zz[r]] = quantise_f64(y[r], qm_exact(a, layer, (4 * gq + r) * S + i));
        }
        const int4 o = reinterpret_cast<const int4 *>(out_slab)[lane];
        reinterpret_cast<int4 *>(a.coeffs + out_base)[lane] = o;
    };
    while (true) {
        step(x0, d0, x2, d2); item += 4; if (item >= last) break;
        step(x1, d1, x0, d0); item += 4; if (item >= last) break;
        step(x2, d2, x1, d1); item += 4; if (item >= last) break;
    }
}
template <bool WANT_DCT>
__device__ __forceinline__ void dct16_body(const Geom &g, const QtGeom &q, const DctArgs &a, long long max_items, unsigned bid, unsigned nb)
{
    __shared__ Dct16Lds L;
    if (g.tiled) dct16_impl<WANT_DCT, true>(L, g, q, a, max_items, bid, nb);
    else dct16_impl<WANT_DCT, false>(L, g, q, a, max_items, bid, nb);
}
template <bool WANT_DCT>
__global__ __launch_bounds__(256) void k_dct16_mfma(Geom g, QtGeom q, DctArgs a, long long max_items)
{
    dct16_body<WANT_DCT>(g, q, a, max_items, blockIdx.x, gridDim.x);
}

template <int S, bool WANT_DCT>
__global__ __launch_bounds__(256) void k_dct_big(Geom g, QtGeom q, DctArgs a, long long max_items)
{
    __shared__ BigTileLds L;
    __shared__ LayerTab lt;
    extern __shared__ int s_pref[];
    dct_prologue(g, q, a, s_pref, lt);
    long long count = s_pref[a.nplanes];
    if (count > max_items) count = max_items;
    const long long wstride = q.work_stride[a.k];
    float *T = a.scratch + (long long)blockIdx.x * S * S;
    for (long long item = blockIdx.x; item < count; item += gridDim.x) {
        const int4 cur = fetch_item(a, wstride, lt, s_pref, item);
        const int b = cur.x / 3, layer = cur.x - b * 3;
        const int w = lt.w[layer], h = lt.h[layer];
        const float *src = a.norm + (long long)b * g.pstride + lt.poff[layer];
        const int hc = min(S, h - cur.z), wc = min(S, w - cur.y);
        const float *D = a.D;
        big_product<S>(L,
            [&](int i, int k) { return D[i * S + k]; },
            [&](int k, int j) { return src[plane_elem(g.tiled, w, cur.z + reflect_pad_idx(k, hc), cur.y + reflect_pad_idx(j, wc))]; },
            [&](int i, int j, float v) { T[i * S + j] = v; });
        big_scratch_sync();
        const long long out_base = (long long)b * q.coeff_stride + lt.coff[layer] + cur.w;
        const int *qm = a.qm[layer];
        big_product<S>(L,
            [&](int i, int k) { return T[i * S + k]; },
            [&](int k, int j) { return D[j * S + k]; },
            [&](int i, int j, float v) {
                const int ridx = i * S + j;
                if (WANT_DCT) a.dct_f32[out_base + ridx] = v;
                a.coeffs[out_base + a.zzinv[ridx]] = quantise(v, qm ? qm[ridx] : 1);
            });
        big_scratch_sync();
    }
}

__device__ __forceinline__ void glds16(const float *g, float *lds_wave_base)
{
    unsigned keep;
    const unsigned dst = __builtin_amdgcn_readfirstlane((unsigned)(size_t)lds_wave_base);
    asm volatile("s_mov_b32 %0, m0\n\ts_mov_b32 m0, %2\n\ts_nop 0\n\tglobal_load_lds_dwordx4 %1, off\n\ts_mov_b32 m0, %0"
                 : "=&s"(keep) : "v"(g), "s"(dst) : "memory");
}
__device__ __forceinline__ void glds4(const float *g, float *lds_wave_base)
{
    unsigned keep;
    const unsigned dst = __builtin_amdgcn_readfirstlane((unsigned)(size_t)lds_wave_base);
    asm volatile("s_mov_b32 %0, m0\n\ts_mov_b32 m0, %2\n\ts_nop 0\n\tglobal_load_lds_dword %1, off\n\ts_mov_b32 m0, %0"
                 : "=&s"(keep) : "v"(g), "s"(dst) : "memory");
}

template <int S>
struct MfmaCfg {
    static constexpr int NT = S / 32;
    static constexpr int TPW = S == 128 ? 2 : 1;
    static constexpr int NWAVES = NT * NT / TPW;
    static constexpr int NTHREADS = NWAVES * 64;
    static constexpr int MINW = S == 32 ? 4 : S == 64 ? 3 : 2;
    static constexpr int NXB = S == 128 ? 1 : 2;
};

__device__ __forceinline__ void glds16_s(const float *base_uniform, unsigned lane_byte_off, float *lds_wave_base)
{
    unsigned keep;
    const unsigned dst = __builtin_amdgcn_readfirstlane((unsigned)(size_t)lds_wave_base);
    const unsigned long long b = (unsigned long long)(size_t)base_uniform;
    const unsigned blo = __builtin_amdgcn_readfirstlane((unsigned)b), bhi = __builtin_amdgcn_readfirstlane((unsigned)(b >> 32));
    const unsigned long long sb = ((unsigned long long)bhi << 32) | blo;
    asm volatile("s_mov_b32 %0, m0\n\ts_mov_b32 m0, %2\n\ts_nop 0\n\tglobal_load_lds_dwordx4 %1, %3\n\ts_mov_b32 m0, %0"
                 : "=&s"(keep) : "v"(lane_byte_off), "s"(dst), "s"(sb) : "memory");
}

template <int S, int NWAVES>
struct XOffsets { unsigned off[S * S / 256 / NWAVES]; int w; };

template <int S, int NWAVES>
__device__ __forceinline__ void dct_x_offsets(XOffsets<S, NWAVES> &xo, int w, int tiled, int wave, int lane)
{
    constexpr int ROWS = 256 / S;
#pragma unroll
    for (int t = 0; t < S * S / 256 / NWAVES; t++) {
        const int chunk = t * NWAVES + wave;
        const int r = chunk * ROWS + lane / (S / 4), c = (lane % (S / 4)) * 4;
        xo.off[t] = (unsigned)plane_elem(tiled, w, r, c) * 4u;
    }
    xo.w = w;
}

template <int S, int NWAVES>
__device__ __forceinline__ void dct_load_x(const float *src, int w, int h, int tiled, const int4 &d, float *sX, int wave, int lane, XOffsets<S, NWAVES> &xo)
{
    constexpr int SS = S * S;
    const int hc = min(S, h - d.z), wc = min(S, w - d.y);
    if (hc == S && wc == S && (w & 3) == 0) {
        if (xo.w != w) dct_x_offsets<S, NWAVES>(xo, w, tiled, wave, lane);
        const float *leaf = src + plane_elem(tiled, w, d.z, d.y);
#pragma unroll
        for (int t = 0; t < SS / 256 / NWAVES; t++) glds16_s(leaf, xo.off[t], sX + (t * NWAVES + wave) * 256);
    } else {
#pragma unroll 4
        for (int t = 0; t < SS / 64 / NWAVES; t++) {
            const int chunk = t * NWAVES + wave;
            const int idx = chunk * 64 + lane;
            const int r = idx / S, c = idx - r * S;
            glds4(src + plane_elem(tiled, w, d.z + reflect_pad_idx(r, hc), d.y + reflect_pad_idx(c, wc)), sX + chunk * 64);
        }
    }
}

__device__ __forceinline__ void lds_barrier() { asm volatile("s_waitcnt lgkmcnt(0)\n\ts_barrier" ::: "memory"); }
template <int N> __device__ __forceinline__ void wait_vmem_but() { asm volatile("s_waitcnt vmcnt(%0)" :: "n"(N) : "memory"); }


template <int S, bool WANT_DCT>
__device__ __forceinline__ void dct_mfma_leaves(const Geom &g, const QtGeom &q, const DctArgs &a, long long max_items, const LeafWork *__restrict__ work ,
                                                unsigned bid, unsigned nb)
{
    using C = MfmaCfg<S>;
    constexpr int NT = C::NT, TPW = C::TPW, NWAVES = C::NWAVES, NTHREADS = C::NTHREADS;
    constexpr int SS = S * S;
    constexpr int NXB = C::NXB;
    constexpr int NCOPY = SS / (NTHREADS * 4);
    constexpr int NYOUNG = NCOPY + (WANT_DCT ? 16 * TPW : 0);
    static_assert(NYOUNG < 60, "vmcnt is a 6-bit counter");
    extern __shared__ __attribute__((aligned(16))) float smem[];
    float *sXb = smem;
    float *sP = smem + NXB * SS;
    int4 *s_desc = reinterpret_cast<int4 *>(smem + (NXB + 1) * SS);
    LayerTab &lt = *reinterpret_cast<LayerTab *>(s_desc + 2 * kDescChunk);
    int *s_pref = reinterpret_cast<int *>(s_desc + 2 * kDescChunk) + (sizeof(LayerTab) + 3) / 4;
    const int tid = threadIdx.x;
    const int wave = tid >> 6, lane = tid & 63;
    const int wj = wave % NT, wi0 = wave / NT;
    const int J0 = wj * 32;
    const int li = lane & 31, lh = lane >> 5;

    float dreg[S / 2];
#pragma unroll
    for (int s = 0; s < S / 2; s++) dreg[s] = a.D[(J0 + li) * S + 2 * s + lh];

    dct_prologue(g, q, a, s_pref, lt);
#pragma unroll
    for (int s = 0; s < S / 2; s++) asm volatile("" : "+v"(dreg[s]));
    long long count = s_pref[a.nplanes];
    if (count > max_items) count = max_items;
    const long long wstride = q.work_stride[a.k];
    const long long step = nb;
    long long item = bid;
    auto load_chunk = [&](long long c) {
        if (tid < kDescChunk) {
            const long long it = (long long)bid + (c * kDescChunk + tid) * step;
            int4 d = make_int4(0, 0, 0, 0);
            if (it < count) d = fetch_item(a, wstride, lt, s_pref, it);
            s_desc[(c & 1) * kDescChunk + tid] = d;
        }
    };
    load_chunk(0);
    load_chunk(1);
    __syncthreads();
    long long k = 0;
    struct LeafU { int plane, x, y, coef; };
    auto uniform = [](const int4 &d) {
        return LeafU{ __builtin_amdgcn_readfirstlane(d.x), __builtin_amdgcn_readfirstlane(d.y), __builtin_amdgcn_readfirstlane(d.z),
                      __builtin_amdgcn_readfirstlane(d.w) };
    };
    auto plane_of = [&](const LeafU &d, int &b, int &layer, int &w, int &h, const float *&src) {
        b = d.plane / 3;
        layer = d.plane - 3 * b;
        w = layer == 0 ? g.w[0] : layer == 1 ? g.w[1] : g.w[2];
        h = layer == 0 ? g.h[0] : layer == 1 ? g.h[1] : g.h[2];
        const long long poff = layer == 0 ? g.poff[0] : layer == 1 ? g.poff[1] : g.poff[2];
        src = a.norm + (long long)b * g.pstride + poff;
    };
    LeafU cur = uniform(s_desc[0]), nxt = uniform(s_desc[1]);
    int pb = 0;
    XOffsets<S, NWAVES> xo;
    xo.w = -1;
    if (NXB == 2 && item < count) {
        int b0, l0, w0, h0;
        const float *src0;
        plane_of(cur, b0, l0, w0, h0, src0);
        dct_load_x<S, NWAVES>(src0, w0, h0, g.tiled, make_int4(cur.plane, cur.x, cur.y, cur.coef), sXb, wave, lane, xo);
        wait_vmem_but<0>();
    }
    float qf[TPW][16];
    int q_layer = -1;
    bool q_slow = false;
    for (; item < count; item += step) {
        int b, layer, lw, lhh;
        const float *src;
        plane_of(cur, b, layer, lw, lhh, src);
        const long long coff = layer == 0 ? q.coeff_off[0] : layer == 1 ? q.coeff_off[1] : q.coeff_off[2];
        const long long out_base = (long long)b * q.coeff_stride + coff + cur.coef;
        float *sX = sXb + pb * SS;
        if (S == 128 || layer != q_layer) {
            const int *qm = layer == 0 ? a.qm[0] : layer == 1 ? a.qm[1] : a.qm[2];
            int qmax = 0;
#pragma unroll
            for (int t = 0; t < TPW; t++)
#pragma unroll
                for (int r = 0; r < 16; r++) {
                    const int qi = qm[((wi0 + t * (NT / TPW)) * 32 + (r & 3) + 8 * (r >> 2) + 4 * lh) * S + J0 + li];
                    qmax = max(qmax, qi);
                    qf[t][r] = (float)qi;
                }
            q_slow = __any(qmax > (1 << 22));
            if (q_slow) {
#pragma unroll
                for (int t = 0; t < TPW; t++)
#pragma unroll
                    for (int r = 0; r < 16; r++) qf[t][r] = __int_as_float(qm[((wi0 + t * (NT / TPW)) * 32 + (r & 3) + 8 * (r >> 2) + 4 * lh) * S + J0 + li]);
            }
            q_layer = layer;
            if (S != 128) {
#pragma unroll
                for (int t = 0; t < TPW; t++)
#pragma unroll
                    for (int r = 0; r < 16; r++) asm volatile("" : "+v"(qf[t][r]));
            }
        }
        if (NXB == 1) {
            dct_load_x<S, NWAVES>(src, lw, lhh, g.tiled, make_int4(cur.plane, cur.x, cur.y, cur.coef), sX, wave, lane, xo);
            wait_vmem_but<0>();
        }
        lds_barrier();
        if (NXB == 2 && item + step < count) {
            int bn, ln, wn, hn;
            const float *srcn;
            plane_of(nxt, bn, ln, wn, hn, srcn);
            dct_load_x<S, NWAVES>(srcn, wn, hn, g.tiled, make_int4(nxt.plane, nxt.x, nxt.y, nxt.coef), sXb + (pb ^ 1) * SS, wave, lane, xo);
        }
        if ((k & (kDescChunk - 1)) == 0 && k > 0) load_chunk(k / kDescChunk + 1);
        floatx16 acc[TPW];
#pragma unroll
        for (int t = 0; t < TPW; t++)
#pragma unroll
            for (int r = 0; r < 16; r++) acc[t][r] = 0.f;
        mfma_chain<S, TPW, kMfmaPF>(sX, (NT / TPW) * 32, wi0 * 32 + li, lh, dreg, acc);
#pragma unroll
        for (int t = 0; t < TPW; t++)
#pragma unroll
            for (int r = 0; r < 16; r++) {
                int row = (r & 3) + 8 * (r >> 2) + 4 * lh;
                sP[((wi0 + t * (NT / TPW)) * 32 + row) * S + J0 + li] = acc[t][r];
            }
        lds_barrier();

#pragma unroll
        for (int t = 0; t < TPW; t++)
#pragma unroll
            for (int r = 0; r < 16; r++) acc[t][r] = 0.f;
        mfma_chain<S, TPW, kMfmaPF>(sP, (NT / TPW) * 32, wi0 * 32 + li, lh, dreg, acc);
        int *sQ = reinterpret_cast<int *>(sX);
        float ymax = 0.f;
#pragma unroll
        for (int t = 0; t < TPW; t++)
#pragma unroll
            for (int r = 0; r < 16; r += 2) ymax = __builtin_fmaxf(__builtin_fmaxf(ymax, __builtin_fabsf(acc[t][r])), __builtin_fabsf(acc[t][r + 1]));
        const bool slow = q_slow || __any(!(ymax < 131072.0f));
#pragma unroll
        for (int t = 0; t < TPW; t++)
#pragma unroll
            for (int r = 0; r < 16; r++) {
                int row = (wi0 + t * (NT / TPW)) * 32 + (r & 3) + 8 * (r >> 2) + 4 * lh;
                if (WANT_DCT) a.dct_f32[out_base + row * S + J0 + li] = acc[t][r];
                const float y = acc[t][r], qq = qf[t][r];
                int v = 0;
                if (q_slow) v = quantise_f64(y, __float_as_int(qq));
                else if (!__all(__builtin_fabsf(y) < 0.499f * qq)) v = slow ? quantise_f64(y, (int)qq) : quantise_f32(y, qq);
                sQ[zigzag_pos<S>(row, J0 + li)] = v;
            }
        lds_barrier();
        for (int idx = tid * 4; idx < SS; idx += NTHREADS * 4)
            *reinterpret_cast<int4 *>(a.coeffs + out_base + idx) = *reinterpret_cast<const int4 *>(sQ + idx);
        if (NXB == 2) wait_vmem_but<NYOUNG>();
        else lds_barrier();
        k++;
        cur = nxt;
        nxt = uniform(s_desc[(k + 1) & (2 * kDescChunk - 1)]);
        pb ^= (NXB - 1);
    }
}

template <int S, bool WANT_DCT>
__global__ __launch_bounds__(MfmaCfg<S>::NTHREADS, MfmaCfg<S>::MINW) void k_dct_mfma(Geom g, QtGeom q, DctArgs a, long long max_items, const LeafWork *__restrict__ work)
{
    dct_mfma_leaves<S, WANT_DCT>(g, q, a, max_items, work, blockIdx.x, gridDim.x);
}

constexpr int kW64Waves = 8;
constexpr int kW64Stride = 68;
struct __attribute__((aligned(16))) Wave64Lds {
    float dop[2][32][64];
    float qT[3][64][kW64Stride];
    unsigned short zT[64][kW64Stride];
    float qlo[3][64][16];
    float qlo16[3][64][4];
    int slab[kW64Waves][1024];
    LayerTab lt;
    int q_slow[4];
};

struct Wave64B { float b[2][4]; };
__device__ __forceinline__ Wave64B wave64_b(const Wave64Lds &L, int s0, int lane)
{
    Wave64B r;
#pragma unroll
    for (int i = 0; i < 4; i++) { r.b[0][i] = L.dop[0][s0 + i][lane]; r.b[1][i] = L.dop[1][s0 + i][lane]; }
    return r;
}

template <bool WANT_DCT>
__global__ __launch_bounds__(kW64Waves * 64, 1) void k_dct64_wave(Geom g, QtGeom q, DctArgs a, long long max_items,
                                                                 const LeafWork *__restrict__ work )
{
    constexpr int S = 64;
    __shared__ Wave64Lds L;
    extern __shared__ int s_pref[];
    const int tid = threadIdx.x;
    const int wave = __builtin_amdgcn_readfirstlane(tid >> 6), lane = tid & 63;
    const int li = lane & 31, lh = lane >> 5;
    {
        constexpr int NT = kW64Waves * 64;
        static_assert((2 * 32 * 64) % NT == 0 && (S * S) % NT == 0, "table loops assume whole rounds");
        float dv[2 * 32 * 64 / NT];
#pragma unroll
        for (int i = 0; i < 2 * 32 * 64 / NT; i++) {
            const int idx = tid + i * NT, row = idx >> 6, kk = idx & 63;
            dv[i] = a.D[row * S + kk];
        }
        int qv[3][S * S / NT];
#pragma unroll
        for (int l = 0; l < 3; l++)
#pragma unroll
            for (int i = 0; i < S * S / NT; i++) qv[l][i] = a.qm[l] ? a.qm[l][tid + i * NT] : 1;
#pragma unroll
        for (int i = 0; i < 2 * 32 * 64 / NT; i++) {
            const int idx = tid + i * NT, row = idx >> 6, kk = idx & 63;
            L.dop[row >> 5][kk >> 1][(kk & 1) * 32 + (row & 31)] = dv[i];
        }
        if (tid < 4) L.q_slow[tid] = 0;
        __syncthreads();
#pragma unroll
        for (int l = 0; l < 3; l++) {
            int qmax = 0;
#pragma unroll
            for (int i = 0; i < S * S / NT; i++) {
                const int idx = tid + i * NT, u = idx >> 6, v = idx & 63;
                qmax = max(qmax, qv[l][i]);
                L.qT[l][v][u] = (float)qv[l][i];
                if (l == 0) L.zT[v][u] = (unsigned short)zigzag_pos<S>(u, v);
            }
            if (qmax > (1 << 22)) L.q_slow[l] = 1;
        }
    }
    __syncthreads();
    for (int idx = tid; idx < 3 * 64 * 16; idx += kW64Waves * 64) {
        const int l = idx >> 10, v = (idx >> 4) & 63, u4 = idx & 15;
        const float *qq = &L.qT[l][v][4 * u4];
        L.qlo[l][v][u4] = 0.499f * __builtin_fminf(__builtin_fminf(qq[0], qq[1]), __builtin_fminf(qq[2], qq[3]));
    }
    __syncthreads();
    for (int idx = tid; idx < 3 * 64 * 4; idx += kW64Waves * 64) {
        const int l = idx >> 8, v = (idx >> 2) & 63, k4 = idx & 3, iu = k4 >> 1, hh = k4 & 1;
        float mn = L.qlo[l][v][8 * iu + hh];
        for (int gq = 1; gq < 4; gq++) mn = __builtin_fminf(mn, L.qlo[l][v][8 * iu + 2 * gq + hh]);
        L.qlo16[l][v][k4] = mn;
    }
    dct_prologue(g, q, a, s_pref, L.lt);
    int count = __builtin_amdgcn_readfirstlane(s_pref[a.nplanes]);
    if ((long long)count > max_items) count = (int)max_items;
    const long long wstride = q.work_stride[a.k];
    const int step = (int)gridDim.x * kW64Waves;
    int item = (int)blockIdx.x * kW64Waves + wave;
    struct LeafU { int plane, x, y, coef; };
    int pl = 0;
    auto leaf_at = [&](int it) {
        if (it >= count) return LeafU{ 0, 0, 0, 0 };
        while (pl + 1 < a.nplanes && __builtin_amdgcn_readfirstlane(s_pref[pl + 1]) <= it) pl++;
        pl = __builtin_amdgcn_readfirstlane(pl);
        const int b = pl / 3, l = pl - 3 * b;
        const long long lw = L.lt.woff[l];
        const long long woff = (long long)(((unsigned long long)(unsigned)__builtin_amdgcn_readfirstlane((int)(lw >> 32)) << 32) |
                                           (unsigned)__builtin_amdgcn_readfirstlane((int)lw));
        const long long idx = (long long)b * wstride + woff + (long long)(it - __builtin_amdgcn_readfirstlane(s_pref[pl]));
        const LeafWork d = work[idx];
        const unsigned xy = (unsigned)__builtin_amdgcn_readfirstlane((int)d.xy);
        return LeafU{ pl, (int)(xy & 0xffffu), (int)(xy >> 16), __builtin_amdgcn_readfirstlane(d.coef) };
    };
    float xr[2][32];
    const int pli = (li & 24) | ((li & 3) << 1) | ((li >> 2) & 1);
    auto load_x = [&](const LeafU &d) {
        const int b = d.plane / 3, layer = d.plane - 3 * b;
        const int w = layer == 0 ? g.w[0] : layer == 1 ? g.w[1] : g.w[2];
        const int h = layer == 0 ? g.h[0] : layer == 1 ? g.h[1] : g.h[2];
        const long long poff = layer == 0 ? g.poff[0] : layer == 1 ? g.poff[1] : g.poff[2];
        const float *src = a.norm + (long long)b * g.pstride + poff;
        const int hc = min(S, h - d.y), wc = min(S, w - d.x);
        typedef const char __attribute__((address_space(1))) *gbytes;
        typedef const float __attribute__((address_space(1))) *gfloat;
        unsigned long long base = (unsigned long long)(size_t)(src + plane_elem(g.tiled, w, d.y, d.x));
        const unsigned rowb = (unsigned)w * 4u;
        if (hc == S && wc == S) {
            const unsigned off = g.tiled ? (unsigned)(pli >> 2) * 64u + (unsigned)(pli & 3) * 4u + (lh ? 16u : 0u) : (lh ? rowb : 0u) + (unsigned)pli * 4u;
            const unsigned second = g.tiled ? 512u : 128u;
            const unsigned long long even_step = g.tiled ? 32ull : 2ull * rowb, odd_step = g.tiled ? 4ull * rowb - 32ull : 2ull * rowb;
#pragma unroll
            for (int s = 0; s < 32; s++) {
                const unsigned blo = __builtin_amdgcn_readfirstlane((unsigned)base), bhi = __builtin_amdgcn_readfirstlane((unsigned)(base >> 32));
                const gbytes rowp = (gbytes)(size_t)(((unsigned long long)bhi << 32) | blo);
                xr[0][s] = *(gfloat)(rowp + off);
                xr[1][s] = *(gfloat)(rowp + (off + second));
                base += (s & 1) ? odd_step : even_step;
            }
        } else {
            const int cc0 = reflect_pad_idx(pli, wc), cc1 = reflect_pad_idx(32 + pli, wc);
            int r = 0, dir = hc > 1 ? 1 : 0;
            auto advance = [&]() {
                r += dir;
                if (r == hc - 1 && dir > 0) dir = -1;
                else if (r == 0 && dir < 0) dir = 1;
            };
#pragma unroll
            for (int s = 0; s < 32; s++) {
                const int r0 = r;
                advance();
                const int r1 = r;
                advance();
                const int rr = lh ? r1 : r0;
                const gfloat plane = (gfloat)(size_t)src;
                xr[0][s] = plane[plane_elem(g.tiled, w, d.y + rr, d.x + cc0)];
                xr[1][s] = plane[plane_elem(g.tiled, w, d.y + rr, d.x + cc1)];
                __builtin_amdgcn_sched_barrier(0);
            }
        }
    };
    if (item >= count) return;
    LeafU cur = leaf_at(item);
    load_x(cur);
    int *slab = L.slab[wave];
    for (; item < count; item += step) {
        const LeafU nxt = leaf_at(item + step);
        const int b = cur.plane / 3, layer = cur.plane - 3 * b;
        const long long coff = layer == 0 ? q.coeff_off[0] : layer == 1 ? q.coeff_off[1] : q.coeff_off[2];
        const long long out_base = (long long)b * q.coeff_stride + coff + cur.coef;
        floatx16 P[2][2];
#pragma unroll
        for (int t = 0; t < 4; t++)
#pragma unroll
            for (int r = 0; r < 16; r++) P[t >> 1][t & 1][r] = 0.f;
        {
            Wave64B bc = wave64_b(L, 0, lane), bn = bc;
#pragma unroll
            for (int s0 = 0; s0 < 32; s0 += 4) {
                if (s0 + 4 < 32) bn = wave64_b(L, s0 + 4, lane);
                __builtin_amdgcn_sched_barrier(0);
#pragma unroll
                for (int i = 0; i < 4; i++) {
                    P[0][0] = __builtin_amdgcn_mfma_f32_32x32x2f32(xr[0][s0 + i], bc.b[0][i], P[0][0], 0, 0, 0);
                    P[0][1] = __builtin_amdgcn_mfma_f32_32x32x2f32(xr[0][s0 + i], bc.b[1][i], P[0][1], 0, 0, 0);
                    P[1][0] = __builtin_amdgcn_mfma_f32_32x32x2f32(xr[1][s0 + i], bc.b[0][i], P[1][0], 0, 0, 0);
                    P[1][1] = __builtin_amdgcn_mfma_f32_32x32x2f32(xr[1][s0 + i], bc.b[1][i], P[1][1], 0, 0, 0);
                }
                __builtin_amdgcn_sched_barrier(0);
                bc = bn;
            }
        }
        if (item + step < count) load_x(nxt);
        __builtin_amdgcn_sched_barrier(0);
        floatx16 Y[2][2];
#pragma unroll
        for (int t = 0; t < 4; t++)
#pragma unroll
            for (int r = 0; r < 16; r++) Y[t >> 1][t & 1][r] = 0.f;
        {
            Wave64B bc = wave64_b(L, 0, lane), bn = bc;
#pragma unroll
            for (int s0 = 0; s0 < 32; s0 += 4) {
                if (s0 + 4 < 32) bn = wave64_b(L, s0 + 4, lane);
                __builtin_amdgcn_sched_barrier(0);
#pragma unroll
                for (int i = 0; i < 4; i++) {
                    const int s = s0 + i;
                    const float a0 = P[s >> 4][0][s & 15], a1 = P[s >> 4][1][s & 15];
                    Y[0][0] = __builtin_amdgcn_mfma_f32_32x32x2f32(a0, bc.b[0][i], Y[0][0], 0, 0, 0);
                    Y[0][1] = __builtin_amdgcn_mfma_f32_32x32x2f32(a0, bc.b[1][i], Y[0][1], 0, 0, 0);
                    Y[1][0] = __builtin_amdgcn_mfma_f32_32x32x2f32(a1, bc.b[0][i], Y[1][0], 0, 0, 0);
                    Y[1][1] = __builtin_amdgcn_mfma_f32_32x32x2f32(a1, bc.b[1][i], Y[1][1], 0, 0, 0);
                }
                __builtin_amdgcn_sched_barrier(0);
                bc = bn;
            }
        }
        const float (*qT)[kW64Stride] = L.qT[layer];
        const float (*qlo)[16] = L.qlo[layer];
        bool redo = L.q_slow[layer] != 0;
        bool upper = false;
#pragma unroll
        for (int c = 0; c < 4; c++) reinterpret_cast<int4 *>(slab)[c * 64 + lane] = make_int4(0, 0, 0, 0);
        int hi_lane = 0;
        if (WANT_DCT) {
#pragma unroll
            for (int t = 0; t < 4; t++)
#pragma unroll
                for (int r = 0; r < 16; r++)
                    a.dct_f32[out_base + (32 * (t >> 1) + 8 * (r >> 2) + 4 * lh + (r & 3)) * S + 32 * (t & 1) + li] = Y[t >> 1][t & 1][r];
        }
        auto tile_max = [&](int iu, int jv) {
            float m16 = 0.f;
#pragma unroll
            for (int r = 0; r < 16; r += 2) m16 = __builtin_fmaxf(__builtin_fmaxf(m16, __builtin_fabsf(Y[iu][jv][r])), __builtin_fabsf(Y[iu][jv][r + 1]));
            return m16;
        };
        auto group_max = [&](int iu, int jv, int gq) {
            return __builtin_fmaxf(__builtin_fmaxf(__builtin_fabsf(Y[iu][jv][4 * gq]), __builtin_fabsf(Y[iu][jv][4 * gq + 1])),
                                   __builtin_fmaxf(__builtin_fabsf(Y[iu][jv][4 * gq + 2]), __builtin_fabsf(Y[iu][jv][4 * gq + 3])));
        };
        auto quantise_group = [&](int iu, int jv, int gq, float m) {
            const int u0 = 32 * iu + 8 * gq + 4 * lh, v = 32 * jv + li;
            if (32 * iu + 32 * jv + 8 * gq >= 45) {
                upper = true;
                return;
            }
            const float4 q4 = *reinterpret_cast<const float4 *>(&qT[v][u0]);
            const uint2 z2 = *reinterpret_cast<const uint2 *>(&L.zT[v][u0]);
            const float qq[4] = { q4.x, q4.y, q4.z, q4.w };
            const int zz[4] = { (int)(z2.x & 0xffffu), (int)(z2.x >> 16), (int)(z2.y & 0xffffu), (int)(z2.y >> 16) };
            hi_lane |= !(m < 131072.0f);
#pragma unroll
            for (int j = 0; j < 4; j++) {
                const int val = quantise_f32(Y[iu][jv][4 * gq + j], qq[j]);
                if (val != 0) {
                    if (zz[j] < 1024) slab[zz[j]] = val;
                    else hi_lane |= 2;
                }
            }
        };
        auto groups_of = [&](int iu, int jv, int first) {
#pragma unroll
            for (int gq = first; gq < 4; gq++) {
                const float m = group_max(iu, jv, gq);
                if (!__all(m < qlo[32 * jv + li][(32 * iu + 8 * gq + 4 * lh) >> 2])) quantise_group(iu, jv, gq, m);
                __builtin_amdgcn_sched_barrier(0);
            }
        };
        quantise_group(0, 0, 0, group_max(0, 0, 0));
        {
            bool zero = true;
#pragma unroll
            for (int gq = 1; gq < 4; gq++) zero = zero && group_max(0, 0, gq) < qlo[li][(8 * gq + 4 * lh) >> 2];
            if (!__all(zero)) groups_of(0, 0, 1);
        }
        {
            const bool zero = tile_max(0, 1) < L.qlo16[layer][32 + li][lh] && tile_max(1, 0) < L.qlo16[layer][li][2 + lh] &&
                              tile_max(1, 1) < L.qlo16[layer][32 + li][2 + lh];
            if (!__all(zero)) {
#pragma unroll
                for (int t = 1; t < 4; t++)
                    if (!__all(tile_max(t >> 1, t & 1) < L.qlo16[layer][32 * (t & 1) + li][2 * (t >> 1) + lh])) groups_of(t >> 1, t & 1, 0);
            }
        }
        if (__any(hi_lane & 1)) redo = true;
        if (__any(hi_lane & 2)) upper = true;
#pragma unroll
        for (int c = 0; c < 4; c++)
            reinterpret_cast<int4 *>(a.coeffs + out_base)[c * 64 + lane] = reinterpret_cast<const int4 *>(slab)[c * 64 + lane];
        if (!upper && !redo) {
#pragma unroll
            for (int c = 0; c < 12; c++) reinterpret_cast<int4 *>(a.coeffs + out_base + 1024)[c * 64 + lane] = make_int4(0, 0, 0, 0);
        } else {
            if (redo) asm volatile("s_waitcnt vmcnt(0)" ::: "memory");
#pragma unroll
            for (int t = 0; t < 4; t++) {
                const int iu = t >> 1, jv = t & 1;
#pragma unroll
                for (int r = 0; r < 16; r++) reinterpret_cast<float *>(slab)[r * 64 + lane] = Y[iu][jv][r];
#pragma unroll 1
                for (int r = 0; r < 16; r++) {
                    const float y = reinterpret_cast<const float *>(slab)[r * 64 + lane];
                    const int u = 32 * iu + 8 * (r >> 2) + 4 * lh + (r & 3), v = 32 * jv + li;
                    const float qq = qT[v][u];
                    const int zz = L.zT[v][u];
                    const bool slow = L.q_slow[layer] != 0 || __any(!(__builtin_fabsf(y) < 131072.0f));
                    const int val = slow ? quantise_f64(y, qm_exact(a, layer, u * S + v)) : quantise_f32(y, qq);
                    if (redo || zz >= 1024) a.coeffs[out_base + zz] = val;
                }
            }
        }
        cur = nxt;
    }
}

template <bool WANT_DCT>
static void launch_dct64_wave(hipStream_t st, const Geom &g, const QtGeom &q, const DctArgs &a, long long max_items)
{
    const size_t pref = (size_t)(a.nplanes + 1) * sizeof(int);
    static int cus = 0;
    if (!cus) {
        int dev = 0;
        hipDeviceProp_t prop;
        cus = (hipGetDevice(&dev) == hipSuccess && hipGetDeviceProperties(&prop, dev) == hipSuccess) ? prop.multiProcessorCount : 256;
    }
    const long long want = (max_items + kW64Waves - 1) / kW64Waves;
    const int blocks = (int)(want < 1 ? 1 : want > cus ? cus : want);
    hipLaunchKernelGGL((k_dct64_wave<WANT_DCT>), dim3(blocks), dim3(kW64Waves * 64), pref, st, g, q, a, max_items,
                       a.work);
}

struct WorkPtrs { LeafWork *w[kMaxSizes]; };

__global__ __launch_bounds__(256) void k_work_from_leaves(const int *__restrict__ leaves, long long n, int bmin_log2, int plane, WorkPtrs wp,
                                                          int *__restrict__ work_count)
{
    long long i = (long long)blockIdx.x * 256 + threadIdx.x;
    if (i >= n) return;
    int4 lf = reinterpret_cast<const int4 *>(leaves)[i];
    int k = (31 - __clz(lf.z)) - bmin_log2;
    if (k < 0 || k >= kMaxSizes || !wp.w[k]) return;
    int pos = atomicAdd(&work_count[plane * kMaxSizes + k], 1);
    wp.w[k][pos] = pack_work(lf.x, lf.y, lf.w);
}

void launch_work_from_leaves(hipStream_t st, const int *leaves, long long n, int bmin, int plane, LeafWork *const *work, int *work_count)
{
    WorkPtrs wp;
    for (int k = 0; k < kMaxSizes; k++) wp.w[k] = work[k];
    if (n <= 0) return;
    hipLaunchKernelGGL(k_work_from_leaves, dim3((unsigned)((n + 255) / 256)), dim3(256), 0, st, leaves, n, ilog2(bmin), plane, wp, work_count);
}

template <int S, bool WANT_DCT>
static void launch_mfma_t(hipStream_t st, const Geom &g, const QtGeom &q, const DctArgs &a, long long max_items)
{
    size_t lds = (size_t)(MfmaCfg<S>::NXB + 1) * S * S * sizeof(float) + 2 * kDescChunk * sizeof(int4) + sizeof(LayerTab) + 8 +
                 (size_t)(a.nplanes + 1) * sizeof(int);
    static size_t attr_lds = 0;
    if (lds > attr_lds) {
        (void)hipFuncSetAttribute(reinterpret_cast<const void *>(&k_dct_mfma<S, WANT_DCT>), hipFuncAttributeMaxDynamicSharedMemorySize, (int)lds);
        attr_lds = lds;
    }
    static size_t occ_lds = ~(size_t)0;
    static int slots = 0;
    if (lds != occ_lds) {
        int per_cu = 0, dev = 0, cus = 256;
        hipDeviceProp_t prop;
        if (hipGetDevice(&dev) == hipSuccess && hipGetDeviceProperties(&prop, dev) == hipSuccess) cus = prop.multiProcessorCount;
        if (hipOccupancyMaxActiveBlocksPerMultiprocessor(&per_cu, k_dct_mfma<S, WANT_DCT>, MfmaCfg<S>::NTHREADS, lds) != hipSuccess || per_cu < 1) per_cu = 1;
        slots = per_cu * cus;
        occ_lds = lds;
    }
    const int blocks = (int)(max_items < slots ? (max_items < 1 ? 1 : max_items) : slots);
    hipLaunchKernelGGL((k_dct_mfma<S, WANT_DCT>), dim3(blocks), dim3(MfmaCfg<S>::NTHREADS), lds, st, g, q, a, max_items,
                       a.work);
}

struct DctMulti {
    DctArgs a[5];
    long long max_items[5];
    int first[6];
};

__global__ __launch_bounds__(256) void k_dct_multi(Geom g, QtGeom q, DctMulti m)
{
    const unsigned b = blockIdx.x;
    if (b < (unsigned)m.first[1]) dct4_body<false>(g, q, m.a[0], m.max_items[0], b - m.first[0], m.first[1] - m.first[0]);
    else if (b < (unsigned)m.first[2]) dct8_body<false>(g, q, m.a[1], m.max_items[1], b - m.first[1], m.first[2] - m.first[1]);
    else if (b < (unsigned)m.first[3]) dct16_body<false>(g, q, m.a[2], m.max_items[2], b - m.first[2], m.first[3] - m.first[2]);
    else if (b < (unsigned)m.first[4]) {
        if (threadIdx.x < MfmaCfg<32>::NTHREADS) dct_mfma_leaves<32, false>(g, q, m.a[3], m.max_items[3], m.a[3].work, b - m.first[3], m.first[4] - m.first[3]);
    } else dct_mfma_leaves<64, false>(g, q, m.a[4], m.max_items[4], m.a[4].work, b - m.first[4], m.first[5] - m.first[4]);
}

int launch_dct_multi(hipStream_t st, const Geom &g, const QtGeom &q, const DctArgs *args, const long long *max_items)
{
    if (q.bmin < 4 || q.bmax > 64 || args[0].dct_f32 || args[0].nplanes > kMaxPlanes) return 1;
    DctMulti m;
    int nb = 0;
    size_t lds = 0;
    for (int slot = 0; slot < 5; slot++) {
        const int size = 4 << slot;
        m.first[slot] = nb;
        if (size < q.bmin || size > q.bmax) { m.a[slot] = args[0]; m.max_items[slot] = 0; continue; }
        const int k = ilog2(size) - ilog2(q.bmin);
        m.a[slot] = args[k];
        m.max_items[slot] = max_items[k];
        if (max_items[k] <= 0) continue;
        auto cap = [&](long long per_block, int hi) { const long long bl = (max_items[k] + per_block - 1) / per_block; return (int)(bl < 1 ? 1 : bl > hi ? hi : bl); };
        const size_t pref = (size_t)(args[k].nplanes + 1) * sizeof(int);
        if (size == 4) { nb += cap(64 * 8, 48); lds = std::max(lds, pref); }
        else if (size == 8) { nb += cap(32, 64); lds = std::max(lds, pref); }
        else if (size == 16) { nb += cap(4, 112); lds = std::max(lds, pref); }
        else {
            const size_t need = size == 32 ? (size_t)(MfmaCfg<32>::NXB + 1) * 32 * 32 * sizeof(float) : (size_t)(MfmaCfg<64>::NXB + 1) * 64 * 64 * sizeof(float);
            lds = std::max(lds, need + 2 * kDescChunk * sizeof(int4) + sizeof(LayerTab) + 8 + pref);
            nb += cap(1, size == 32 ? 96 : 192);
        }
    }
    m.first[5] = nb;
    if (nb == 0) return 0;
    static size_t attr_lds = 0;
    if (lds > attr_lds) {
        (void)hipFuncSetAttribute(reinterpret_cast<const void *>(&k_dct_multi), hipFuncAttributeMaxDynamicSharedMemorySize, (int)lds);
        attr_lds = lds;
    }
    hipLaunchKernelGGL(k_dct_multi, dim3((unsigned)nb), dim3(256), lds, st, g, q, m);
    return 0;
}

int launch_dct(hipStream_t st, int size, const Geom &g, const QtGeom &q, const DctArgs &a, long long max_items, const Tuning &t)
{
    if (max_items <= 0) return 0;
    if (a.nplanes > kMaxPlanes) return -1;
    const size_t pref = (size_t)(a.nplanes + 1) * sizeof(int);
    const int small_wgs = t.dct_small_workgroups;
    auto cap = [&](long long per_block, int hi) {
        long long b = (max_items + per_block - 1) / per_block;
        if (small_wgs > 0 && size <= 16) hi = small_wgs;
        return (int)(b < 1 ? 1 : b > hi ? hi : b);
    };
    const bool wd = a.dct_f32 != nullptr;
#define AEJ_SMALL(S, PER, HI)                                                                                              \
    if (wd) hipLaunchKernelGGL((k_dct_small<S, true>), dim3(cap(PER, HI)), dim3(256), pref, st, g, q, a, max_items);       \
    else hipLaunchKernelGGL((k_dct_small<S, false>), dim3(cap(PER, HI)), dim3(256), pref, st, g, q, a, max_items)
#define AEJ_MFMA(S)                                                     \
    if (wd) launch_mfma_t<S, true>(st, g, q, a, max_items);              \
    else launch_mfma_t<S, false>(st, g, q, a, max_items)
    switch (size) {
    case 2: AEJ_SMALL(2, 128, 2048); break;
    case 4:
        if (wd) hipLaunchKernelGGL((k_dct4<true>), dim3(cap(64 * 8, 8192)), dim3(256), pref, st, g, q, a, max_items);
        else hipLaunchKernelGGL((k_dct4<false>), dim3(cap(64 * 8, 8192)), dim3(256), pref, st, g, q, a, max_items);
        break;
    case 8:
        if (wd) hipLaunchKernelGGL((k_dct8_shfl<true>), dim3(cap(32, 4096)), dim3(256), pref, st, g, q, a, max_items);
        else hipLaunchKernelGGL((k_dct8_shfl<false>), dim3(cap(32, 4096)), dim3(256), pref, st, g, q, a, max_items);
        break;
    case 16:
        if (wd) hipLaunchKernelGGL((k_dct16_mfma<true>), dim3(cap(4, 2048)), dim3(256), pref, st, g, q, a, max_items);
        else hipLaunchKernelGGL((k_dct16_mfma<false>), dim3(cap(4, 2048)), dim3(256), pref, st, g, q, a, max_items);
        break;
    case 32: AEJ_MFMA(32); break;
    case 64: {
        const bool force_four = t.dct64_kernel == 4, force_wave = t.dct64_kernel == 1;
        const bool tiny = max_items < 2048;
        if (wd || force_four || ((a.crowded || tiny) && !force_wave)) { AEJ_MFMA(64); }
        else launch_dct64_wave<false>(st, g, q, a, max_items);
        break;
    }
    case 128: AEJ_MFMA(128); break;
#define AEJ_BIG(S)                                                                                                               \
    if (!a.scratch) return -1;                                    \
    if (wd) hipLaunchKernelGGL((k_dct_big<S, true>), dim3(cap(1, big_blocks(S))), dim3(256), pref, st, g, q, a, max_items);      \
    else hipLaunchKernelGGL((k_dct_big<S, false>), dim3(cap(1, big_blocks(S))), dim3(256), pref, st, g, q, a, max_items)
    case 256: AEJ_BIG(256); break;
    case 512: AEJ_BIG(512); break;
    case 1024: AEJ_BIG(1024); break;
#undef AEJ_BIG
    default: return -1;
    }
#undef AEJ_SMALL
#undef AEJ_MFMA
    return 0;
}

}
```

### include/aej.h

```cpp
#ifndef AEJ_H
#define AEJ_H

#include <stddef.h>
#include <stdint.h>

#ifdef __cplusplus
extern "C" {
#endif

#define AEJ_ABI_VERSION 3

#if defined(__GNUC__)
#define AEJ_API __attribute__((visibility("default")))
#else
#define AEJ_API
#endif

typedef struct aej_ctx aej_ctx;

typedef enum aej_status {
    AEJ_OK = 0,
    AEJ_ERR_ARG = -1,
    AEJ_ERR_HIP = -2,
    AEJ_ERR_STATE = -3,
    AEJ_ERR_CAPACITY = -4,
    AEJ_ERR_UNSUPPORTED = -5
} aej_status;

typedef enum aej_space {
    AEJ_YCBCR = 0, AEJ_YCOCG = 1, AEJ_YCOCG_R = 2, AEJ_OKLAB = 3, AEJ_ICTCP = 4, AEJ_ICACB = 5, AEJ_JZAZBZ = 6,
    AEJ_XYZ = 7
} aej_space;

#define AEJ_MAX_SIZES 8

typedef struct aej_plan {
    int32_t batch, H, W;
    int32_t layer_h[3], layer_w[3];
    int32_t root_size[3];
    int64_t coeff_off[3], coeff_stride;
    int64_t leaf_off[3], leaf_stride;
    int64_t state_off[3], state_stride;
    uint64_t workspace_bytes;
} aej_plan;

AEJ_API int aej_abi_version(void);
AEJ_API aej_ctx *aej_create(int device, void *hip_stream );
AEJ_API void aej_destroy(aej_ctx *ctx);
AEJ_API const char *aej_last_error(aej_ctx *ctx);
AEJ_API int aej_synchronize(aej_ctx *ctx);
AEJ_API int aej_set_stream(aej_ctx *ctx, void *hip_stream);

enum {
    AEJ_STAGE_CLEAR = 0, AEJ_STAGE_COLOR_PLANES, AEJ_STAGE_CLAHE_LUT, AEJ_STAGE_CLAHE_BLUR, AEJ_STAGE_THRESHOLDS,
    AEJ_STAGE_SOBEL_NMS, AEJ_STAGE_HYSTERESIS, AEJ_STAGE_QUADTREE, AEJ_STAGE_DCT_2, AEJ_STAGE_DCT_4, AEJ_STAGE_DCT_8,
    AEJ_STAGE_DCT_16, AEJ_STAGE_DCT_32, AEJ_STAGE_DCT_64, AEJ_STAGE_DCT_128, AEJ_STAGE_DCT_256, AEJ_STAGE_DCT_512, AEJ_STAGE_DCT_1024,
    AEJ_N_STAGES
};
AEJ_API int aej_get_hysteresis_stats(aej_ctx *ctx, int64_t *out_host);
AEJ_API int aej_set_graph_mode(aej_ctx *ctx, int mode);
AEJ_API int aej_set_sub_batches(aej_ctx *ctx, int n);
AEJ_API int aej_set_hw_queues(aej_ctx *ctx, int n);
AEJ_API int aej_get_schedule_host(aej_ctx *ctx, int batch, int H, int W, int32_t *out_host);
AEJ_API int aej_set_option(aej_ctx *ctx, const char *name, int64_t value);
AEJ_API int aej_get_option(aej_ctx *ctx, const char *name, int64_t *value_host);
AEJ_API int aej_encode_batch_begin(aej_ctx *ctx, const void *rgb, int rgb_is_u8, int batch, int H, int W, int32_t *coeffs, int32_t *leaves,
                                   uint8_t *states, int64_t *counts, float *dct_f32, void *workspace, uint64_t workspace_bytes);
AEJ_API int aej_encode_batch_end(aej_ctx *ctx);
AEJ_API int64_t aej_get_split_calls(aej_ctx *ctx);
AEJ_API int aej_get_graph_stats(aej_ctx *ctx, int64_t *out_host);
AEJ_API int aej_set_profiling(aej_ctx *ctx, int enable);
AEJ_API int aej_get_stage_ms(aej_ctx *ctx, float *ms_host );
AEJ_API const char *aej_stage_name(int stage);

AEJ_API int aej_set_settings(aej_ctx *ctx, int space, int bmin, int bmax, const int32_t *qmats_host);

AEJ_API int aej_encode_plan(aej_ctx *ctx, int batch, int H, int W, aej_plan *plan_host);

AEJ_API int aej_encode_batch(aej_ctx *ctx, const float *rgb, int batch, int H, int W,
                     int32_t *coeffs, int32_t *leaves, uint8_t *states, int64_t *counts,
                     float *dct_f32, void *workspace, uint64_t workspace_bytes);

AEJ_API int aej_encode_batch_u8(aej_ctx *ctx, const uint8_t *rgb_u8, int batch, int H, int W,
                     int32_t *coeffs, int32_t *leaves, uint8_t *states, int64_t *counts,
                     float *dct_f32, void *workspace, uint64_t workspace_bytes);

enum { AEJ_METRIC_PSNR = 1, AEJ_METRIC_SSIM = 2, AEJ_METRIC_MS_SSIM = 4 };
AEJ_API uint64_t aej_metrics_workspace_bytes(int batch, int H, int W);
AEJ_API int aej_metrics_batch(aej_ctx *ctx, const float *img_a, const float *img_b, int batch, int H, int W, int which,
                      double *out, void *workspace, uint64_t workspace_bytes);

AEJ_API uint64_t aej_lpips_weights_bytes(void);
AEJ_API int64_t aej_lpips_param_count(void);
AEJ_API int aej_lpips_pack_weights_host(const float *params, int64_t n_params, void *packed_host);
AEJ_API uint64_t aej_lpips_features_bytes(int batch, int H, int W);
AEJ_API uint64_t aej_lpips_workspace_bytes(int batch, int H, int W);
AEJ_API int aej_lpips_features(aej_ctx *ctx, const void *weights, const float *img, int batch, int H, int W, float *feats,
                               void *workspace, uint64_t workspace_bytes);
AEJ_API int aej_lpips_batch(aej_ctx *ctx, const void *weights, const float *img_a, const float *feats_a, const float *img_b, int batch,
                            int H, int W, double *out, void *workspace, uint64_t workspace_bytes);


AEJ_API int aej_color_convert(aej_ctx *ctx, int space, const float *rgb, float *out, int64_t n);

AEJ_API int aej_color_planes(aej_ctx *ctx, const float *rgb, int batch, int H, int W, float *planes_raw,
                     float *planes_norm, uint8_t *planes_u8);

AEJ_API uint64_t aej_canny_workspace_bytes(int H, int W);
typedef struct aej_canny_params {
    double canny_low_ratio, canny_high_ratio;
    double clahe_clip_limit;
    double bilateral_sigma_color, bilateral_sigma_space;
    int use_l2_gradient;
} aej_canny_params;
AEJ_API int aej_set_canny_params(aej_ctx *ctx, const aej_canny_params *params);
AEJ_API int aej_canny(aej_ctx *ctx, const float *plane, int H, int W, uint8_t *edge, uint8_t *stages,
              int32_t *thresholds, void *workspace, uint64_t workspace_bytes);

AEJ_API uint64_t aej_quadtree_workspace_bytes(int H, int W, int min_size, int max_size);
AEJ_API int aej_quadtree_capacity(int H, int W, int min_size, int max_size, int64_t *leaf_cap, int64_t *state_cap,
                          int64_t *coeff_cap);
AEJ_API int aej_quadtree(aej_ctx *ctx, const uint8_t *edge, int H, int W, int min_size, int max_size,
                 int32_t *leaves, uint8_t *states, int64_t *counts, void *workspace, uint64_t workspace_bytes);

AEJ_API int aej_dct_quant_zigzag(aej_ctx *ctx, const float *norm, int H, int W, int layer, const int32_t *leaves,
                         int64_t n_leaves, int32_t *coeffs, float *dct_f32);

#define AEJ_DEFLATE_HIST_BINS 320
#define AEJ_DEFLATE_TABLE_WORDS 448
AEJ_API uint64_t aej_deflate_stream_bound(uint64_t raw_bytes);
AEJ_API uint64_t aej_deflate_workspace_bytes(aej_ctx *ctx, int batch, int H, int W);
AEJ_API int aej_deflate_histogram(aej_ctx *ctx, const int32_t *coeffs, const int64_t *counts, int batch, int H, int W, int32_t *hist, void *workspace,
                                  uint64_t workspace_bytes);
AEJ_API int aej_deflate_build_tables(const int32_t *hist_host, const int32_t *cover_all, uint32_t *tables_host);
AEJ_API int aej_deflate_batch(aej_ctx *ctx, const int32_t *coeffs, const int64_t *counts, int batch, int H, int W, const uint32_t *tables, int reuse_parse,
                              uint8_t *streams, uint64_t stream_stride, int64_t *sizes, void *workspace, uint64_t workspace_bytes);

AEJ_API int aej_pack_u8_levels_host(const float *rgb_host, int64_t n, uint8_t *u8_host, int threads);

AEJ_API uint64_t aej_decode_workspace_bytes(aej_ctx *ctx, int batch, int H, int W);
AEJ_API int aej_decode_batch(aej_ctx *ctx, const int32_t *coeffs, const int32_t *leaves, const int64_t *counts, int batch, int H,
                             int W, float *rgb_out, void *workspace, uint64_t workspace_bytes);
AEJ_API int aej_decode_batch_tables(aej_ctx *ctx, const int32_t *coeffs, const int32_t *leaves, const int64_t *counts, int batch, int H, int W,
                                    const int32_t *qmats_dev, float *rgb_out, void *workspace, uint64_t workspace_bytes);

AEJ_API int aej_requantise_batch(aej_ctx *ctx, const float *dct_f32, const int32_t *leaves, const int64_t *counts, int batch, int H, int W,
                                 int n_sets, const int32_t *qmats_dev, int32_t *coeffs_out, uint64_t set_stride_elems);
AEJ_API int aej_color_convert_inverse(aej_ctx *ctx, int space, const float *in, float *out_rgb, int64_t n);
AEJ_API int64_t aej_leaf_positions_host(const int32_t *sizes_host, int64_t n, int root, int H, int W, int32_t *xy_host);

enum {
    AEJ_INFLATE_OK = 0, AEJ_INFLATE_BAD_HEADER = 1 , AEJ_INFLATE_BAD_BLOCK_TYPE = 2,
    AEJ_INFLATE_BAD_CODE_LENGTHS = 3 ,
    AEJ_INFLATE_BAD_SYMBOL = 4 ,
    AEJ_INFLATE_DISTANCE_TOO_FAR = 5, AEJ_INFLATE_STORED_LENGTH = 6 , AEJ_INFLATE_TRUNCATED = 7,
    AEJ_INFLATE_OVER_CAPACITY = 8, AEJ_INFLATE_ADLER = 9, AEJ_INFLATE_BAD_ARG = 10
};
AEJ_API int aej_inflate_batch(aej_ctx *ctx, const uint8_t *src, const int64_t *streams, int n, uint8_t *dst, uint64_t dst_bytes,
                              int64_t *out_bytes, int32_t *status);
enum {
    AEJ_HEADER_OK = 0, AEJ_HEADER_TOO_MANY_LEAVES = 1, AEJ_HEADER_BAD_SIZE = 2 ,
    AEJ_HEADER_NO_TILING = 3, AEJ_HEADER_COEFF_COUNT = 4 , AEJ_HEADER_BAD_ARG = 5
};
AEJ_API uint64_t aej_decode_headers_workspace_bytes(aej_ctx *ctx, int batch, int H, int W);
AEJ_API int aej_decode_headers(aej_ctx *ctx, const uint8_t *states, const int64_t *layers, const int64_t *inflated_bytes, int batch, int H, int W,
                               int32_t *leaves, int64_t *counts, int32_t *status, void *workspace, uint64_t workspace_bytes);

AEJ_API uint64_t aej_jfif_workspace_bytes(int batch, int H, int W, int n_q);
AEJ_API int aej_jfif_headers_host(int quality, int H, int W, uint8_t *out_host, int capacity);
AEJ_API int aej_jfif_encode_batch(aej_ctx *ctx, const uint8_t *rgb, int batch, int H, int W, int n_q, const int32_t *qualities_host, uint8_t *out,
                                  uint64_t out_capacity, int64_t *offsets, int64_t *lengths, uint64_t *total_host, void *workspace,
                                  uint64_t workspace_bytes);
AEJ_API int aej_jfif_recon_batch(aej_ctx *ctx, int batch, int H, int W, int n_q, uint8_t *rgb_out, void *workspace, uint64_t workspace_bytes);
AEJ_API uint64_t aej_jfif_workspace_bytes_opt(int batch, int H, int W, int n_q, int subsampling, int optimize);
AEJ_API int aej_jfif_headers_host_opt(int quality, int H, int W, int subsampling, uint8_t *out_host, int capacity);
AEJ_API int aej_jfif_huffman_host(const int64_t *counts_host, uint8_t *bits_host, uint8_t *huffval_host, int capacity);
AEJ_API int aej_jfif_encode_batch_opt(aej_ctx *ctx, const uint8_t *rgb, int batch, int H, int W, int n_q, const int32_t *qualities_host,
                                      int subsampling, int optimize, uint8_t *out, uint64_t out_capacity, int64_t *offsets, int64_t *lengths,
                                      uint64_t *total_host, void *workspace, uint64_t workspace_bytes);
AEJ_API int aej_jfif_recon_batch_opt(aej_ctx *ctx, int batch, int H, int W, int n_q, int subsampling, int optimize, uint8_t *rgb_out,
                                     void *workspace, uint64_t workspace_bytes);

AEJ_API uint64_t aej_jfif_workspace_bytes_prog(int batch, int H, int W, int n_q, int subsampling);
AEJ_API int aej_jfif_encode_batch_prog(aej_ctx *ctx, const uint8_t *rgb, int batch, int H, int W, int n_q, const int32_t *qualities_host,
                                       int subsampling, uint8_t *out, uint64_t out_capacity, int64_t *offsets, int64_t *lengths,
                                       uint64_t *total_host, void *workspace, uint64_t workspace_bytes);
AEJ_API int aej_jfif_recon_batch_prog(aej_ctx *ctx, int batch, int H, int W, int n_q, int subsampling, uint8_t *rgb_out, void *workspace,
                                      uint64_t workspace_bytes);

enum {
    AEJ_JPEGDEC_OK = 0, AEJ_JPEGDEC_TRUNCATED = 1 , AEJ_JPEGDEC_BAD_CODE = 2 ,
    AEJ_JPEGDEC_RUN_PAST_63 = 3 , AEJ_JPEGDEC_BAD_DC = 4 ,
    AEJ_JPEGDEC_BAD_RESTART = 5 ,
    AEJ_JPEGDEC_COEF_RANGE = 6
};
typedef struct aej_jpegdec_huff {
    uint16_t lut[512];
    int32_t maxcode[18];
    int32_t valoff[18];
    uint8_t vals[256];
} aej_jpegdec_huff;
typedef struct aej_jpegdec_desc {
    int32_t width, height;
    int32_t ncomp;
    int32_t hs, vs;
    int32_t mcux, mcuy;
    int32_t blocks_per_mcu;
    int32_t restart_interval;
    int32_t n_segments;
    int32_t sof;
    int32_t precision16;
    uint8_t comp_id[4], comp_h[4], comp_v[4], comp_tq[4];
    uint16_t qt[3][64];
    aej_jpegdec_huff dc[3], ac[3];
    int64_t scan_offset, scan_length;
} aej_jpegdec_desc;
AEJ_API int aej_jpegdec_parse_host(const uint8_t *data_host, uint64_t nbytes, aej_jpegdec_desc *desc_host, char *msg, int msg_capacity);
// ... 112 lines not shown
```

Before: 83900 MP/s.

## Skip DCT second-pass MFMA for 32-row bands provably quantising to zero

Precomputes per-band energy thresholds from the DCT basis norm and the minimum quantiser per 32-row band for 64 and 128 blocks. After the first DCT pass, each wave computes column energy into LDS, and bands whose bound guarantees every coefficient quantises to zero skip the second MFMA chain and write zeros directly. This applies to both the generic MFMA leaf kernel and the dedicated 64-wide kernel. It adds an LDS norm buffer, extra reductions and branching, and depends on a conservative bound to stay exact.

Result: no change. 83760 MP/s (-0.2%).

```diff
diff --git a/adaptive_edge_aware_jpeg_amd/_lib.py b/adaptive_edge_aware_jpeg_amd/_lib.py
--- a/adaptive_edge_aware_jpeg_amd/_lib.py
+++ b/adaptive_edge_aware_jpeg_amd/_lib.py
@@ -151,6 +151,8 @@
     "aej_get_schedule_host": (_I, [_P, _I, _I, _I, _P]),
     "aej_set_option": (_I, [_P, ctypes.c_char_p, _I64]),
     "aej_get_option": (_I, [_P, ctypes.c_char_p, _P]),
+    "aej_dct_zero_thresholds_host": (_I, [_P, _I, _I, _P]),
+    "aej_dct_zero_thresholds_for_host": (_I, [_I, _P, _P]),
     "aej_test_fail_after_stage": (_I, [_P, _I]),
     "aej_encode_batch_begin": (_I, [_P, _P, _I, _I, _I, _I, _P, _P, _P, _P, _P, _P, _U64]),
     "aej_encode_batch_end": (_I, [_P]),
diff --git a/adaptive_edge_aware_jpeg_amd/csrc/aej_common.h b/adaptive_edge_aware_jpeg_amd/csrc/aej_common.h
--- a/adaptive_edge_aware_jpeg_amd/csrc/aej_common.h
+++ b/adaptive_edge_aware_jpeg_amd/csrc/aej_common.h
@@ -52,6 +52,7 @@
     int dct_small_workgroups = 0;
     int sobel_lds = 0;
     int dct_multi = 1;
+    int dct_zero_skip = 1;
     int sobel_xcd = 1;
 };
 
diff --git a/adaptive_edge_aware_jpeg_amd/csrc/aej_ctx.h b/adaptive_edge_aware_jpeg_amd/csrc/aej_ctx.h
--- a/adaptive_edge_aware_jpeg_amd/csrc/aej_ctx.h
+++ b/adaptive_edge_aware_jpeg_amd/csrc/aej_ctx.h
@@ -30,6 +30,8 @@
     const int *d_zzinv[aej::kMaxSizes] = {};
     const int *d_zz[aej::kMaxSizes] = {};
     const int *d_qm[3][aej::kMaxSizes] = {};
+    const float *d_zthr[3][aej::kMaxSizes] = {};
+    std::vector<float> h_zthr[3][aej::kMaxSizes];
     int *d_check = nullptr;
     const float *d_space_w = nullptr, *d_color_w = nullptr;
     float *d_bilateral = nullptr;
diff --git a/adaptive_edge_aware_jpeg_amd/csrc/aej_launch.h b/adaptive_edge_aware_jpeg_amd/csrc/aej_launch.h
--- a/adaptive_edge_aware_jpeg_amd/csrc/aej_launch.h
+++ b/adaptive_edge_aware_jpeg_amd/csrc/aej_launch.h
@@ -84,6 +84,7 @@
     const float *D;
     const int *zzinv;
     const int *qm[3];
+    const float *zthr[3] = {};
     int crowded = 0;
 };
 int launch_dct(hipStream_t st, int size, const Geom &g, const QtGeom &q, const DctArgs &a, long long max_items, const Tuning &t);
diff --git a/adaptive_edge_aware_jpeg_amd/csrc/api.hip b/adaptive_edge_aware_jpeg_amd/csrc/api.hip
--- a/adaptive_edge_aware_jpeg_amd/csrc/api.hip
+++ b/adaptive_edge_aware_jpeg_amd/csrc/api.hip
@@ -221,6 +221,61 @@
     }
 }
 
+static void dct_basis(int s, std::vector<float> &D)
+{
+    D.resize((size_t)s * s);
+    for (int u = 0; u < s; u++) {
+        double alpha = u == 0 ? sqrt(1.0 / (double)s) : sqrt(2.0 / (double)s);
+        for (int n = 0; n < s; n++) D[(size_t)u * s + n] = (float)(alpha * cos(3.14159265358979323846 * (double)(2 * n + 1) * (double)u / (2.0 * (double)s)));
+    }
+}
+
+static void zero_thresholds(int s, const float *D, const int32_t *q, std::vector<float> &out)
+{
+    const int nb = s / 32;
+    out.assign((size_t)nb * s, 0.f);
+    double dmax = 0.0;
+    for (int v = 0; v < s; v++) {
+        double n2 = 0.0;
+        for (int k = 0; k < s; k++) n2 += (double)D[(size_t)v * s + k] * (double)D[(size_t)v * s + k];
+        dmax = std::max(dmax, sqrt(n2));
+    }
+    const double e = (double)s / 8388608.0;
+    const double c = std::min(0.45, 0.45 / ((1.0 + e) * (1.0 + e) * dmax));
+    for (int i = 0; i < s * s; i++) if (q[i] > (1 << 22)) return;
+    for (int b = 0; b < nb; b++)
+        for (int u = 0; u < s; u++) {
+            int qmin = q[(size_t)u * s + 32 * b];
+            for (int v = 32 * b; v < 32 * b + 32; v++) qmin = std::min(qmin, q[(size_t)u * s + v]);
+            const double t = c * (double)qmin * c * (double)qmin;
+            float f = (float)t;
+            if ((double)f > t) f = nextafterf(f, 0.f);
+            out[(size_t)b * s + u] = f;
+        }
+}
+
+extern "C" int aej_dct_zero_thresholds_for_host(int size, const int32_t *q_host, float *out_host)
+{
+    if ((size != 64 && size != 128) || !q_host || !out_host) return AEJ_ERR_ARG;
+    for (int i = 0; i < size * size; i++) if (q_host[i] < 1) return AEJ_ERR_ARG;
+    std::vector<float> D, t;
+    dct_basis(size, D);
+    zero_thresholds(size, D.data(), q_host, t);
+    memcpy(out_host, t.data(), t.size() * sizeof(float));
+    return 0;
+}
+
+extern "C" int aej_dct_zero_thresholds_host(aej_ctx *ctx, int layer, int size, float *out_host)
+{
+    if (!ctx || !out_host) return AEJ_ERR_ARG;
+    if (!ctx->has_settings) return fail(ctx, AEJ_ERR_ARG, "aej_dct_zero_thresholds_host: no settings");
+    if (layer < 0 || layer > 2 || (size != 64 && size != 128) || size < ctx->bmin || size > ctx->bmax)
+        return fail(ctx, AEJ_ERR_ARG, "aej_dct_zero_thresholds_host: layer %d, size %d: layers 0..2 and the sizes 64 / 128 of the settings have a table", layer, size);
+    const std::vector<float> &t = ctx->h_zthr[layer][ilog2(size) - ilog2(ctx->bmin)];
+    memcpy(out_host, t.data(), t.size() * sizeof(float));
+    return 0;
+}
+
 extern "C" int aej_set_settings(aej_ctx *ctx, int space, int bmin, int bmax, const int32_t *qmats_host)
 {
     AEJ_TRY(enter(ctx, __func__));
@@ -242,16 +297,14 @@
         memcpy(blob.data() + o, p, bytes);
         return o;
     };
-    size_t oD[kMaxSizes], oZ[kMaxSizes], oZf[kMaxSizes], oQ[3][kMaxSizes];
+    size_t oD[kMaxSizes], oZ[kMaxSizes], oZf[kMaxSizes], oQ[3][kMaxSizes], oT[3][kMaxSizes];
+    std::vector<float> zt[3][kMaxSizes];
     int k = 0;
     size_t qpos = 0;
     std::vector<size_t> qoff_layer_size;
     for (int s = bmin; s <= bmax; s *= 2, k++) {
-        std::vector<float> D((size_t)s * s);
-        for (int u = 0; u < s; u++) {
-            double alpha = u == 0 ? sqrt(1.0 / (double)s) : sqrt(2.0 / (double)s);
-            for (int n = 0; n < s; n++) D[(size_t)u * s + n] = (float)(alpha * cos(3.14159265358979323846 * (double)(2 * n + 1) * (double)u / (2.0 * (double)s)));
-        }
+        std::vector<float> D;
+        dct_basis(s, D);
         oD[k] = put(D.data(), D.size() * 4);
         std::vector<int> zz, inv((size_t)s * s);
         zigzag_order(s, zz);
@@ -265,6 +318,10 @@
             for (int i = 0; i < s * s; i++)
                 if (qmats_host[qpos + i] < 1) return fail(ctx, AEJ_ERR_ARG, "quantisation matrix entries must be >= 1");
             oQ[l][k] = put(qmats_host + qpos, (size_t)s * s * 4);
+            if (s == 64 || s == 128) {
+                zero_thresholds(s, reinterpret_cast<const float *>(blob.data() + oD[k]), qmats_host + qpos, zt[l][k]);
+                oT[l][k] = put(zt[l][k].data(), zt[l][k].size() * 4);
+            }
             qpos += (size_t)s * s;
         }
     }
@@ -277,13 +334,16 @@
     char *base = static_cast<char *>(ctx->tables);
     for (int i = 0; i < kMaxSizes; i++) {
         ctx->d_D[i] = nullptr; ctx->d_zzinv[i] = nullptr; ctx->d_zz[i] = nullptr;
-        for (int l = 0; l < 3; l++) ctx->d_qm[l][i] = nullptr;
+        for (int l = 0; l < 3; l++) { ctx->d_qm[l][i] = nullptr; ctx->d_zthr[l][i] = nullptr; ctx->h_zthr[l][i].clear(); }
     }
     for (int i = 0; i < nsizes; i++) {
         ctx->d_D[i] = reinterpret_cast<const float *>(base + oD[i]);
         ctx->d_zzinv[i] = reinterpret_cast<const int *>(base + oZ[i]);
         ctx->d_zz[i] = reinterpret_cast<const int *>(base + oZf[i]);
-        for (int l = 0; l < 3; l++) ctx->d_qm[l][i] = reinterpret_cast<const int *>(base + oQ[l][i]);
+        for (int l = 0; l < 3; l++) {
+            ctx->d_qm[l][i] = reinterpret_cast<const int *>(base + oQ[l][i]);
+            if (!zt[l][i].empty()) { ctx->d_zthr[l][i] = reinterpret_cast<const float *>(base + oT[l][i]); ctx->h_zthr[l][i] = zt[l][i]; }
+        }
     }
     ctx->d_check = reinterpret_cast<int *>(base + oCheck);
     ctx->space = space; ctx->bmin = bmin; ctx->bmax = bmax; ctx->nsizes = nsizes;
@@ -352,6 +412,7 @@
     { "sobel_lds", &aej::Tuning::sobel_lds, nullptr, 0, 1, true },
     { "sobel_xcd", &aej::Tuning::sobel_xcd, nullptr, 0, 1, true },
     { "dct_multi", &aej::Tuning::dct_multi, nullptr, 0, 1, true },
+    { "dct_zero_skip", &aej::Tuning::dct_zero_skip, nullptr, 0, 1, true },
     { "sub_chain", nullptr, &aej_ctx::sub_chain, -1, 3, false },
     { "jpegdec_subseq_bits", nullptr, &aej_ctx::jd_subseq_bits, 32, 1 << 20, false },
 };
diff --git a/adaptive_edge_aware_jpeg_amd/csrc/api_encode.hip b/adaptive_edge_aware_jpeg_amd/csrc/api_encode.hip
--- a/adaptive_edge_aware_jpeg_amd/csrc/api_encode.hip
+++ b/adaptive_edge_aware_jpeg_amd/csrc/api_encode.hip
@@ -310,6 +310,7 @@
         a.D = ctx->d_D[k]; a.zzinv = ctx->d_zzinv[k];
         a.crowded = ctx->dct_crowded;
         for (int l = 0; l < 3; l++) a.qm[l] = ctx->d_qm[l][k];
+        if (ctx->tune.dct_zero_skip) for (int l = 0; l < 3; l++) a.zthr[l] = ctx->d_zthr[l][k];
     }
     const bool one_launch = ctx->tune.dct_multi && !ctx->profiling && (long long)g.B * g.H * g.W <= kGraphAutoPixels;
     if (!(one_launch && launch_dct_multi(st, g, q, args, w.qt.qb.work_cap) == 0)) {
@@ -819,6 +820,7 @@
             a.scratch = big_scratch_floats(ctx->bmax) ? reinterpret_cast<float *>(scratch + big_off) : nullptr;
             a.D = ctx->d_D[k]; a.zzinv = ctx->d_zzinv[k];
             for (int l = 0; l < 3; l++) a.qm[l] = ctx->d_qm[l][k];
+            if (ctx->tune.dct_zero_skip) for (int l = 0; l < 3; l++) a.zthr[l] = ctx->d_zthr[l][k];
             if (launch_dct(st, s, g, q, a, n_leaves, ctx->tune)) { e = hipErrorInvalidValue; break; }
         }
         if (e == hipSuccess) e = hipGetLastError();
diff --git a/adaptive_edge_aware_jpeg_amd/csrc/dct.hip b/adaptive_edge_aware_jpeg_amd/csrc/dct.hip
--- a/adaptive_edge_aware_jpeg_amd/csrc/dct.hip
+++ b/adaptive_edge_aware_jpeg_amd/csrc/dct.hip
@@ -681,6 +681,9 @@
     static constexpr int NTHREADS = NWAVES * 64;
     static constexpr int MINW = S == 32 ? 4 : S == 64 ? 3 : 2;
     static constexpr int NXB = S == 128 ? 1 : 2;
+    static constexpr bool ZSKIP = S >= 64;
+    static constexpr int NNORM = ZSKIP ? 4 * S : 0;
+    static constexpr int LDS_FLOATS = (NXB + 1) * S * S + NNORM;
 };
 
 __device__ __forceinline__ void glds16_s(const float *base_uniform, unsigned lane_byte_off, float *lds_wave_base)
@@ -734,6 +737,8 @@
 __device__ __forceinline__ void lds_barrier() { asm volatile("s_waitcnt lgkmcnt(0)\n\ts_barrier" ::: "memory"); }
 template <int N> __device__ __forceinline__ void wait_vmem_but() { asm volatile("s_waitcnt vmcnt(%0)" :: "n"(N) : "memory"); }
 
+
+template <int V> struct IntC { static constexpr int value = V; };
 
 template <int S, bool WANT_DCT>
 __device__ __forceinline__ void dct_mfma_leaves(const Geom &g, const QtGeom &q, const DctArgs &a, long long max_items, const LeafWork *__restrict__ work ,
@@ -749,12 +754,18 @@
     extern __shared__ __attribute__((aligned(16))) float smem[];
     float *sXb = smem;
     float *sP = smem + NXB * SS;
-    int4 *s_desc = reinterpret_cast<int4 *>(smem + (NXB + 1) * SS);
+    float *sN = smem + (NXB + 1) * SS;
+    int4 *s_desc = reinterpret_cast<int4 *>(smem + C::LDS_FLOATS);
     LayerTab &lt = *reinterpret_cast<LayerTab *>(s_desc + 2 * kDescChunk);
     int *s_pref = reinterpret_cast<int *>(s_desc + 2 * kDescChunk) + (sizeof(LayerTab) + 3) / 4;
     const int tid = threadIdx.x;
     const int wave = tid >> 6, lane = tid & 63;
     const int wj = wave % NT, wi0 = wave / NT;
+    const int wi0s = __builtin_amdgcn_readfirstlane(wi0);
+    constexpr bool ZS = C::ZSKIP && !WANT_DCT;
+    constexpr bool ALT = ZS && S == 64;
+    constexpr int NQ = ALT ? 2 : TPW;
+    const bool zon = ZS && a.zthr[0] != nullptr;
     const int J0 = wj * 32;
     const int li = lane & 31, lh = lane >> 5;
 
@@ -806,7 +817,10 @@
         dct_load_x<S, NWAVES>(src0, w0, h0, g.tiled, make_int4(cur.plane, cur.x, cur.y, cur.coef), sXb, wave, lane, xo);
         wait_vmem_but<0>();
     }
-    float qf[TPW][16];
+    float qf[NQ][16];
+    float zthr[TPW];
+#pragma unroll
+    for (int t = 0; t < TPW; t++) zthr[t] = 0.f;
     int q_layer = -1;
     bool q_slow = false;
     for (; item < count; item += step) {
@@ -818,28 +832,36 @@
         float *sX = sXb + pb * SS;
         if (S == 128 || layer != q_layer) {
             const int *qm = layer == 0 ? a.qm[0] : layer == 1 ? a.qm[1] : a.qm[2];
+            auto qrow = [&](int t, int r) { return ((ALT ? t : wi0 + t * (NT / TPW)) * 32 + (r & 3) + 8 * (r >> 2) + 4 * lh) * S + J0 + li; };
             int qmax = 0;
 #pragma unroll
-            for (int t = 0; t < TPW; t++)
+            for (int t = 0; t < NQ; t++)
 #pragma unroll
                 for (int r = 0; r < 16; r++) {
-                    const int qi = qm[((wi0 + t * (NT / TPW)) * 32 + (r & 3) + 8 * (r >> 2) + 4 * lh) * S + J0 + li];
+                    const int qi = qm[qrow(t, r)];
                     qmax = max(qmax, qi);
                     qf[t][r] = (float)qi;
                 }
+            if (zon) {
+                const float *zt = layer == 0 ? a.zthr[0] : layer == 1 ? a.zthr[1] : a.zthr[2];
+#pragma unroll
+                for (int t = 0; t < TPW; t++) zthr[t] = zt[wj * S + (ALT ? 1 : wi0 + t * (NT / TPW)) * 32 + li];
+            }
             q_slow = __any(qmax > (1 << 22));
             if (q_slow) {
 #pragma unroll
-                for (int t = 0; t < TPW; t++)
-#pragma unroll
-                    for (int r = 0; r < 16; r++) qf[t][r] = __int_as_float(qm[((wi0 + t * (NT / TPW)) * 32 + (r & 3) + 8 * (r >> 2) + 4 * lh) * S + J0 + li]);
+                for (int t = 0; t < NQ; t++)
+#pragma unroll
+                    for (int r = 0; r < 16; r++) qf[t][r] = __int_as_float(qm[qrow(t, r)]);
             }
             q_layer = layer;
             if (S != 128) {
 #pragma unroll
-                for (int t = 0; t < TPW; t++)
+                for (int t = 0; t < NQ; t++)
 #pragma unroll
                     for (int r = 0; r < 16; r++) asm volatile("" : "+v"(qf[t][r]));
+#pragma unroll
+                for (int t = 0; t < TPW; t++) asm volatile("" : "+v"(zthr[t]));
             }
         }
         if (NXB == 1) {
@@ -867,13 +889,44 @@
                 int row = (r & 3) + 8 * (r >> 2) + 4 * lh;
                 sP[((wi0 + t * (NT / TPW)) * 32 + row) * S + J0 + li] = acc[t][r];
             }
+        if (zon) {
+            float n2 = 0.f;
+#pragma unroll
+            for (int t = 0; t < TPW; t++)
+#pragma unroll
+                for (int r = 0; r < 16; r++) n2 = __builtin_fmaf(acc[t][r], acc[t][r], n2);
+            sN[(wi0 * 2 + lh) * S + J0 + li] = n2;
+        }
         lds_barrier();
 
+        const int ui0 = ALT && zon ? wi0s ^ (int)(k & 1) : wi0s;
+        bool skip[TPW];
+        bool any_skip = false;
+#pragma unroll
+        for (int t = 0; t < TPW; t++) {
+            skip[t] = false;
+            const int ub = ui0 + t * (NT / TPW);
+            if (zon && !q_slow && ub >= 1) {
+                const int u = ub * 32 + li;
+                const float n2 = (sN[u] + sN[S + u]) + (sN[2 * S + u] + sN[3 * S + u]);
+                skip[t] = !__any(!(n2 < zthr[t]));
+                any_skip = any_skip || skip[t];
+            }
+        }
 #pragma unroll
         for (int t = 0; t < TPW; t++)
 #pragma unroll
             for (int r = 0; r < 16; r++) acc[t][r] = 0.f;
-        mfma_chain<S, TPW, kMfmaPF>(sP, (NT / TPW) * 32, wi0 * 32 + li, lh, dreg, acc);
+        if (!any_skip) mfma_chain<S, TPW, kMfmaPF>(sP, (NT / TPW) * 32, ui0 * 32 + li, lh, dreg, acc);
+        else if (TPW > 1) {
+#pragma unroll
+            for (int t = 0; t < TPW; t++)
+                if (!skip[t]) {
+                    floatx16 one[1] = { acc[t] };
+                    mfma_chain<S, 1, kMfmaPF>(sP, 0, (ui0 + t * (NT / TPW)) * 32 + li, lh, dreg, one);
+                    acc[t] = one[0];
+                }
+        }
         int *sQ = reinterpret_cast<int *>(sX);
         float ymax = 0.f;
 #pragma unroll
@@ -881,18 +934,30 @@
 #pragma unroll
             for (int r = 0; r < 16; r += 2) ymax = __builtin_fmaxf(__builtin_fmaxf(ymax, __builtin_fabsf(acc[t][r])), __builtin_fabsf(acc[t][r + 1]));
         const bool slow = q_slow || __any(!(ymax < 131072.0f));
-#pragma unroll
-        for (int t = 0; t < TPW; t++)
-#pragma unroll
-            for (int r = 0; r < 16; r++) {
-                int row = (wi0 + t * (NT / TPW)) * 32 + (r & 3) + 8 * (r >> 2) + 4 * lh;
-                if (WANT_DCT) a.dct_f32[out_base + row * S + J0 + li] = acc[t][r];
-                const float y = acc[t][r], qq = qf[t][r];
-                int v = 0;
-                if (q_slow) v = quantise_f64(y, __float_as_int(qq));
-                else if (!__all(__builtin_fabsf(y) < 0.499f * qq)) v = slow ? quantise_f64(y, (int)qq) : quantise_f32(y, qq);
-                sQ[zigzag_pos<S>(row, J0 + li)] = v;
-            }
+        auto emit = [&](auto qs) {
+            constexpr int QS = decltype(qs)::value;
+#pragma unroll
+            for (int t = 0; t < TPW; t++) {
+                const int row0 = (ALT ? QS : ui0 + t * (NT / TPW)) * 32 + 4 * lh;
+                if (skip[t]) {
+#pragma unroll
+                    for (int r = 0; r < 16; r++) sQ[zigzag_pos<S>(row0 + (r & 3) + 8 * (r >> 2), J0 + li)] = 0;
+                    continue;
+                }
+#pragma unroll
+                for (int r = 0; r < 16; r++) {
+                    int row = row0 + (r & 3) + 8 * (r >> 2);
+                    if (WANT_DCT) a.dct_f32[out_base + row * S + J0 + li] = acc[t][r];
+                    const float y = acc[t][r], qq = qf[ALT ? QS : t][r];
+                    int v = 0;
+                    if (q_slow) v = quantise_f64(y, __float_as_int(qq));
+                    else if (!__all(__builtin_fabsf(y) < 0.499f * qq)) v = slow ? quantise_f64(y, (int)qq) : quantise_f32(y, qq);
+                    sQ[zigzag_pos<S>(row, J0 + li)] = v;
+                }
+            }
+        };
+        if (ALT && ui0) emit(IntC<1>());
+        else emit(IntC<0>());
         lds_barrier();
         for (int idx = tid * 4; idx < SS; idx += NTHREADS * 4)
             *reinterpret_cast<int4 *>(a.coeffs + out_base + idx) = *reinterpret_cast<const int4 *>(sQ + idx);
@@ -919,6 +984,7 @@
     unsigned short zT[64][kW64Stride];
     float qlo[3][64][16];
     float qlo16[3][64][4];
+    float zthr[3][32];
     int slab[kW64Waves][1024];
     LayerTab lt;
     int q_slow[4];
@@ -989,6 +1055,11 @@
         float mn = L.qlo[l][v][8 * iu + hh];
         for (int gq = 1; gq < 4; gq++) mn = __builtin_fminf(mn, L.qlo[l][v][8 * iu + 2 * gq + hh]);
         L.qlo16[l][v][k4] = mn;
+    }
+    const bool zon = !WANT_DCT && a.zthr[0] != nullptr;
+    if (tid < 3 * 32) {
+        const int l = tid >> 5, i = tid & 31;
+        L.zthr[l][i] = zon && a.zthr[l] ? __builtin_fminf(a.zthr[l][32 + i], a.zthr[l][S + 32 + i]) : 0.f;
     }
     dct_prologue(g, q, a, s_pref, L.lt);
     int count = __builtin_amdgcn_readfirstlane(s_pref[a.nplanes]);
@@ -1089,6 +1160,16 @@
                 bc = bn;
             }
         }
+        bool lower = true;
+        if (zon && __builtin_amdgcn_readfirstlane(L.q_slow[layer]) == 0) {
+            float n2 = 0.f;
+#pragma unroll
+            for (int wi = 0; wi < 2; wi++)
+#pragma unroll
+                for (int r = 0; r < 16; r++) n2 = __builtin_fmaf(P[wi][1][r], P[wi][1][r], n2);
+            n2 += __shfl_xor(n2, 32);
+            lower = __any(!(n2 < L.zthr[layer][li]));
+        }
         if (item + step < count) load_x(nxt);
         __builtin_amdgcn_sched_barrier(0);
         floatx16 Y[2][2];
@@ -1096,7 +1177,8 @@
         for (int t = 0; t < 4; t++)
 #pragma unroll
             for (int r = 0; r < 16; r++) Y[t >> 1][t & 1][r] = 0.f;
-        {
+        auto chain2 = [&](auto lo) {
+            constexpr bool LO = decltype(lo)::value != 0;
             Wave64B bc = wave64_b(L, 0, lane), bn = bc;
 #pragma unroll
             for (int s0 = 0; s0 < 32; s0 += 4) {
@@ -1108,13 +1190,17 @@
                     const float a0 = P[s >> 4][0][s & 15], a1 = P[s >> 4][1][s & 15];
                     Y[0][0] = __builtin_amdgcn_mfma_f32_32x32x2f32(a0, bc.b[0][i], Y[0][0], 0, 0, 0);
                     Y[0][1] = __builtin_amdgcn_mfma_f32_32x32x2f32(a0, bc.b[1][i], Y[0][1], 0, 0, 0);
-                    Y[1][0] = __builtin_amdgcn_mfma_f32_32x32x2f32(a1, bc.b[0][i], Y[1][0], 0, 0, 0);
-                    Y[1][1] = __builtin_amdgcn_mfma_f32_32x32x2f32(a1, bc.b[1][i], Y[1][1], 0, 0, 0);
+                    if (LO) {
+                        Y[1][0] = __builtin_amdgcn_mfma_f32_32x32x2f32(a1, bc.b[0][i], Y[1][0], 0, 0, 0);
+                        Y[1][1] = __builtin_amdgcn_mfma_f32_32x32x2f32(a1, bc.b[1][i], Y[1][1], 0, 0, 0);
+                    }
                 }
                 __builtin_amdgcn_sched_barrier(0);
                 bc = bn;
             }
-        }
+        };
+        if (lower) chain2(IntC<1>());
+        else chain2(IntC<0>());
         const float (*qT)[kW64Stride] = L.qT[layer];
         const float (*qlo)[16] = L.qlo[layer];
         bool redo = L.q_slow[layer] != 0;
@@ -1255,7 +1341,7 @@
 template <int S, bool WANT_DCT>
 static void launch_mfma_t(hipStream_t st, const Geom &g, const QtGeom &q, const DctArgs &a, long long max_items)
 {
-    size_t lds = (size_t)(MfmaCfg<S>::NXB + 1) * S * S * sizeof(float) + 2 * kDescChunk * sizeof(int4) + sizeof(LayerTab) + 8 +
+    size_t lds = (size_t)MfmaCfg<S>::LDS_FLOATS * sizeof(float) + 2 * kDescChunk * sizeof(int4) + sizeof(LayerTab) + 8 +
                  (size_t)(a.nplanes + 1) * sizeof(int);
     static size_t attr_lds = 0;
     if (lds > attr_lds) {
@@ -1314,7 +1400,7 @@
         else if (size == 8) { nb += cap(32, 64); lds = std::max(lds, pref); }
         else if (size == 16) { nb += cap(4, 112); lds = std::max(lds, pref); }
         else {
-            const size_t need = size == 32 ? (size_t)(MfmaCfg<32>::NXB + 1) * 32 * 32 * sizeof(float) : (size_t)(MfmaCfg<64>::NXB + 1) * 64 * 64 * sizeof(float);
+            const size_t need = (size == 32 ? MfmaCfg<32>::LDS_FLOATS : MfmaCfg<64>::LDS_FLOATS) * sizeof(float);
             lds = std::max(lds, need + 2 * kDescChunk * sizeof(int4) + sizeof(LayerTab) + 8 + pref);
             nb += cap(1, size == 32 ? 96 : 192);
         }
diff --git a/include/aej.h b/include/aej.h
--- a/include/aej.h
+++ b/include/aej.h
@@ -63,6 +63,8 @@
 AEJ_API int aej_set_hw_queues(aej_ctx *ctx, int n);
 AEJ_API int aej_get_schedule_host(aej_ctx *ctx, int batch, int H, int W, int32_t *out_host);
 AEJ_API int aej_set_option(aej_ctx *ctx, const char *name, int64_t value);
+AEJ_API int aej_dct_zero_thresholds_host(aej_ctx *ctx, int layer, int size, float *out_host);
+AEJ_API int aej_dct_zero_thresholds_for_host(int size, const int32_t *q_host, float *out_host);
 AEJ_API int aej_get_option(aej_ctx *ctx, const char *name, int64_t *value_host);
 AEJ_API int aej_encode_batch_begin(aej_ctx *ctx, const void *rgb, int rgb_is_u8, int batch, int H, int W, int32_t *coeffs, int32_t *leaves,
                                    uint8_t *states, int64_t *counts, float *dct_f32, void *workspace, uint64_t workspace_bytes);
```
